# manhtuando97/two-stage-gnn

Hardware: AMD Instinct MI355X
Metric: graphs/sec fwd+bwd, DD batch=32 SAGE-3L h=128 (higher is better)
Workload: dtype f32

## Files before the change

include/tsgnn.h:

```cpp
#ifndef TSGNN_H
#define TSGNN_H
#include <stdint.h>

typedef struct ihipStream_t* tsgnn_stream_t;

#ifdef __cplusplus
extern "C" {
#endif

#define TSGNN_ABI_VERSION 2
int tsgnn_abi_version(void);
const char* tsgnn_strerror(int code);
const char* tsgnn_last_kernel(void);


int tsgnn_scan_workspace_ints(int64_t n, int64_t* ws_ints);
int tsgnn_exclusive_scan_i32(const int* in, int64_t n, int* out, int* ws, tsgnn_stream_t stream);

int tsgnn_row_maps(const int* graph_ptr, int B, int64_t n_rows, int* row_graph, int* row_slot,
                   tsgnn_stream_t stream);

int tsgnn_dense_adj_count(const float* adj, int B, int nmax, const int* graph_ptr, const int* row_graph,
                          int64_t n_rows, int* row_cnt, tsgnn_stream_t stream);
int tsgnn_dense_adj_fill(const float* adj, int B, int nmax, const int* graph_ptr, const int* row_graph,
// ... 41 lines not shown
int tsgnn_collate_pool_submit(tsgnn_collate_pool* pool, const int64_t* ds_graph_ptr, const int64_t* ds_rowptr, const int64_t* ds_col,
                              const int64_t* ds_node_label, const int64_t* ds_graph_label, const int64_t* ids, int B, int nmax,
                              int64_t row_cap, int64_t edge_cap, int ell_w, int64_t tail_cap, int32_t* staging, int64_t* out,
                              void* after_event, int64_t* ticket);
int tsgnn_collate_pool_submit_ack(tsgnn_collate_pool* pool, const int64_t* ds_graph_ptr, const int64_t* ds_rowptr, const int64_t* ds_col,
                                  const int64_t* ds_node_label, const int64_t* ds_graph_label, const int64_t* ids, int B, int nmax,
                                  int64_t row_cap, int64_t edge_cap, int ell_w, int64_t tail_cap, int32_t* staging, int64_t* out,
                                  const int64_t* host_ack, int64_t ack_target, int seq, int64_t* ticket);
int tsgnn_collate_pool_wait(tsgnn_collate_pool* pool, int64_t ticket);
int tsgnn_collate_pool_destroy(tsgnn_collate_pool* pool);

int tsgnn_csr_transpose(const int* rowptr, const int* col, const float* val, int64_t n_rows, int64_t n_cols,
                        int64_t nnz, int* rowptr_t, int* col_t, float* val_t, int* src_e, int* cnt_ws,
                        int* scan_ws, tsgnn_stream_t stream);


int tsgnn_csr_spmm_f32(const int* rowptr, const int* col, const float* val, const float* self_w,
                       const float* x, int64_t ldx, float* y, int64_t ldy, int64_t n_rows, int feat,
                       float self_scalar, int relu_in, int accumulate, tsgnn_stream_t stream);

int tsgnn_csr_to_ell(const int* rowptr, const int* col, int64_t n_rows, int W, int* ell, int* tail_cnt, tsgnn_stream_t stream);
int tsgnn_csr_tail_fill(const int* rowptr, const int* col, const int* tail_ptr, int64_t n_rows, int W, int* tail_col,
                        tsgnn_stream_t stream);
int tsgnn_ell_spmm_f32(const int* ell, int W, const float* x, int64_t ldx, float* y, int64_t ldy, int64_t n_rows, int feat,
                       float self_scalar, tsgnn_stream_t stream);

int tsgnn_gcn_norm_f32(const int* rowptr, const int* col, const float* val, int64_t n_rows, float self_fill,
                       float* dinv, float* val_out, float* self_w, tsgnn_stream_t stream);

int tsgnn_sddmm_rows_f32(const int* rowptr, const int* col, const float* dy, int64_t lddy, const float* x, int64_t ldx,
                         int64_t n_rows, int feat, float* dval, float* dself, tsgnn_stream_t stream);


int tsgnn_gemm_f32(const float* A, int64_t sam, int64_t sak, const float* B, int64_t sbk, int64_t sbn, float* C,
                   int64_t scm, int64_t scn, int M, int N, int K, int batch, int64_t stride_a, int64_t stride_b,
                   int64_t stride_c, const int* seg_ptr, int ragged, int max_seg, float alpha, int accumulate,
                   tsgnn_stream_t stream);
int tsgnn_gemm_splitk_plan(int M, int N, int K, int* ksplit, int64_t* ws_floats);
int tsgnn_gemm_splitk_f32(const float* A, int64_t sam, int64_t sak, const float* B, int64_t sbk, int64_t sbn,
                          float* C, int M, int N, int K, int ksplit, float* ws, int accumulate,
                          tsgnn_stream_t stream);
int tsgnn_linear_wgrad_plan(int64_t rows, int K_in, int N, int64_t ldz, int64_t lddu, int* nslab, int64_t* rows_per_slab,
                            int64_t* ws_floats);
int tsgnn_linear_wgrad_f32(const float* z, int64_t ldz, const float* du, int64_t lddu, int64_t rows, int K_in, int N, int nslab,
                           int64_t rows_per_slab, int64_t bias_only_rows, float* ws, float* dw, float* db, tsgnn_stream_t stream);
int tsgnn_wgrad_reduce_sets_blocks(const int64_t* desc);
int tsgnn_wgrad_reduce_sets_f32(const int64_t* desc, float* normparts, float* step_state, tsgnn_stream_t stream);
int tsgnn_wgrad_reduce_multi_f32(const float* ws0, int nslab0, int K0, int N0, float* dw0, float* db0, const float* ws1, int nslab1,
                                 int K1, int N1, float* dw1, float* db1, const float* ws2, int nslab2, int K2, int N2, float* dw2,
                                 float* db2, const float* ws3, int nslab3, int K3, int N3, float* dw3, float* db3,
                                 float* normparts, float* step_state, tsgnn_stream_t stream);
int tsgnn_wgrad_blocks_plan(int64_t rows, int K_in, int N, int64_t ldz, int64_t lddu, int* nslab, int64_t* rows_per_slab,
                            int64_t* ws_floats);
int tsgnn_wgrad_blocks_f32(const float* z, int64_t ldz, const float* du, int64_t lddu, int64_t rows, int K_in, int N, int nslab,
                           int64_t rows_per_slab, float* ws, float* dw, int64_t lddw, tsgnn_stream_t stream);
int tsgnn_wgrad_blocks_oi_f32(const float* z, int64_t ldz, const float* du, int64_t lddu, int64_t rows, int K_in, int N, int nslab,
                              int64_t rows_per_slab, float* ws, float* dw_oi, int64_t lddw, float* db, tsgnn_stream_t stream);
int tsgnn_ragged_tn_f32(const float* s_mat, int64_t lds_, const float* x, int64_t ldx, int K, int N, const int* slab_row_ptr,
                        int nslab, const int* seg_slab_ptr, int nseg, float* ws, float* out, tsgnn_stream_t stream);
int tsgnn_ragged_tn_direct_supported(int K, int64_t max_rows);
int tsgnn_ragged_tn_direct_f32(const float* s_mat, int64_t lds_, int K, const int* graph_ptr, int B, const float* x0, int64_t ldx0,
                               int N0, float* out0, const float* x1, int64_t ldx1, int N1, float* out1, tsgnn_stream_t stream);
int tsgnn_ragged_tn_direct_ro_f32(const float* s_mat, int64_t lds_, int K, const int* graph_ptr, int B, const float* x0, int64_t ldx0,
                                  int N0, float* out0, const float* x1, int64_t ldx1, int N1, float* out1, float* ro_out,
                                  int64_t ro_ldo, int* ro_arg, int nmax, int64_t n_real, int ghost_zero, tsgnn_stream_t stream);
int tsgnn_wgrad_narrow_plan(int64_t rows, int K_in, int N, int64_t* ws_floats);
int tsgnn_wgrad_narrow_f32(const float* z, int64_t ldz, const float* du, int64_t lddu, int64_t rows, int K_in, int N, float* ws,
                           float* dwb, tsgnn_stream_t stream);
int tsgnn_colsum_f32(const float* x, int64_t ld, int64_t rows, int F, float* out, float* ws, int accumulate,
                     tsgnn_stream_t stream);

int tsgnn_linear_l2norm_f32(const float* z, int64_t ldz, const float* w, int64_t ldw, const float* bias, float* v,
                            int64_t ldv, float* rinv, int64_t rows, int K, int N, int normalize,
                            tsgnn_stream_t stream);
int tsgnn_rowgemm_supported(const float* a, int64_t lda, const float* b, int64_t ldb, const float* c, int64_t ldc, int K, int N,
                            int trans_b);
int tsgnn_rowgemm_f32(const float* a, int64_t lda, const float* b, int64_t ldb, int trans_b, const float* bias, float* c,
                      int64_t ldc, float* rinv, int64_t rows, int K, int N, int normalize, int64_t fill_rows,
                      tsgnn_stream_t stream);
int tsgnn_panel_blocks(int64_t rows, int panel_units);
int tsgnn_gather_rowgemm_f32(const int* ell, int ell_w, const int* tail_ptr, const int* tail_col, const float* x, int64_t ldx, const float* b, int64_t ldb, int trans_b,
                             const float* bias, float* c, int64_t ldc, float* rinv, float* zout, int64_t ldz, int64_t rows, int K,
                             int N, int normalize, int64_t fill_rows, tsgnn_stream_t stream);
int tsgnn_gather_rowgemm_st_f32(const int* ell, int ell_w, const int* tail_ptr, const int* tail_col, const float* x, int64_t ldx, const float* b, int64_t ldb, const float* bias,
                                float* c, int64_t ldc, float* rinv, float* zout, int64_t ldz, int64_t rows, int K, int N,
                                int64_t fill_rows, const int* row_slot, unsigned long long* sums, float* ghost, int panel_units,
                                const int64_t* pack_desc, tsgnn_stream_t stream);
int tsgnn_sage_layer_fwd_bn_f32(const int* ell, int ell_w, const int* tail_ptr, const int* tail_col, const float* x, int64_t ldx, const float* w, int64_t ldw, const float* bias,
                                float* v, int64_t ldv, float* rinv, float* zout, int64_t ldz, int64_t rows, int K, int64_t fill_rows,
                                const int* graph_ptr, const int* slot_count, int B, int nslots, int n_ghost, unsigned long long* packed,
                                unsigned long long* packed_out, const int* row_graph, const unsigned long long* sums_in,
                                const float* ghost_in, float* mean_out, float* rstd_out, const int* row_slot,
                                unsigned long long* sums_out, float* ghost_out, const int* ro_map, int ro_map_ch, int panel_units,
                                const float* w_img, tsgnn_stream_t stream);
int tsgnn_sage_layer_fwd_bn_plan(int64_t rows, int64_t fill_rows, int B, int nslots, int panel_units, int* ro_ch, int* n_gemm,
                                 int* n_full);
int tsgnn_sage_layer_fwd_f32(const int* ell, int ell_w, const int* tail_ptr, const int* tail_col, const float* x, int64_t ldx, const float* w, int64_t ldw, const float* bias,
                             float* v, int64_t ldv, float* rinv, float* zout, int64_t ldz, int64_t rows, int K, int64_t fill_rows,
                             const int* graph_ptr, int B, int nslots, int n_ghost, unsigned long long* packed, tsgnn_stream_t stream);
int tsgnn_sage_layer_fwd_ro_f32(const int* ell, int ell_w, const int* tail_ptr, const int* tail_col, const float* x, int64_t ldx, const float* w, int64_t ldw, const float* bias,
                                float* v, int64_t ldv, float* rinv, float* zout, int64_t ldz, int64_t rows, int K, int64_t fill_rows,
                                const int* graph_ptr, int B, int nslots, int n_ghost, unsigned long long* packed,
                                unsigned long long* packed_out, const int* row_graph, tsgnn_stream_t stream);
int tsgnn_sage_layer_bwd_f32(const int* ell, int ell_w, const int* tail_ptr, const int* tail_col, const float* du, int64_t lddu, const float* w, int64_t ldw, float* dxs,
                             int64_t lddxs, const float* z, int64_t ldz, int64_t rows, int nslab, int64_t rows_per_slab,
                             int64_t bias_only_rows, float* ws, int panel_units, const float* w_img, tsgnn_stream_t stream);
int tsgnn_l2norm_bwd_f32(const float* v, int64_t ldv, const float* dv, int64_t lddv, const float* rinv, float* du,
                         int64_t lddu, int64_t rows, int F, tsgnn_stream_t stream);


int tsgnn_bn_slots_fwd_f32(const int* graph_ptr, const int* slot_count, const int* row_slot, int B, int nmax,
                           int64_t n_real, int n_ghost, const float* v, int64_t ldv, int F, int relu, int bn,
                           float* mean, float* rstd, float* y, int64_t ldy, tsgnn_stream_t stream);
int tsgnn_bn_slots_bwd_f32(const int* graph_ptr, const int* slot_count, const int* row_slot, int B, int nmax,
                           int64_t n_real, int n_ghost, const float* v, int64_t ldv, const float* dy, int64_t lddy, int F,
                           int relu, int bn, const float* mean, const float* rstd, float* m1, float* m2, float* dv,
                           int64_t lddv, tsgnn_stream_t stream);

int tsgnn_row_ln_fwd_f32(const float* v, int64_t ldv, int64_t rows, int F, int relu, float* mean, float* rstd, float* y, int64_t ldy,
                         tsgnn_stream_t stream);
int tsgnn_row_ln_bwd_f32(const float* v, int64_t ldv, const float* dy, int64_t lddy, int64_t rows, int F, int relu, const float* mean,
                         const float* rstd, float* dv, int64_t lddv, tsgnn_stream_t stream);

int tsgnn_row_post_bwd_f32(const int* row_graph, int B, int64_t n_real, int64_t rows, const float* v, int64_t ldv, const float* dxs,
                           int64_t lddxs, const float* dout, int64_t ldo, const int* arg, int F, int relu, int ln, const float* mean,
                           const float* rstd, const float* rinv, float* du, int64_t lddu, tsgnn_stream_t stream);

int tsgnn_row_post_nodes_bwd_f32(int64_t n_real, int64_t rows, const float* v, int64_t ldv, const float* dxs, int64_t lddxs,
                                 const float* dnode, int64_t lddn, int ghost_zero, int F, int relu, int ln, const float* mean,
                                 const float* rstd, const float* rinv, float* du, int64_t lddu, tsgnn_stream_t stream);

int tsgnn_readout_max_ws_words(int B, int nmax, int F);
int tsgnn_readout_max_fwd_f32(const int* graph_ptr, const int* slot_count, int B, int nmax, int64_t n_real, int n_ghost,
                              const float* x, int64_t ldx, int F, int relu, unsigned long long* packed_ws, float* out,
                              int64_t ldo, int* arg, tsgnn_stream_t stream);
int tsgnn_readout_max_bwd_f32(const float* dout, int64_t ldo, const int* arg, int B, int F, const float* x, int64_t ldx_in,
                              int relu, int64_t n_real, float* dx, int64_t ldx, tsgnn_stream_t stream);
int tsgnn_readout_max_bwd_rows_f32(const float* dout, int64_t ldo, const int* arg, const int* row_graph, int F, int64_t rows,
                                   int64_t rows_total, const float* add, int64_t ldadd, float* dx, int64_t ldx, tsgnn_stream_t stream);

int tsgnn_pack_rows_f32(const float* src, int nmax, int F, const int* row_graph, const int* row_slot, int64_t n_real,
                        float* dst, int64_t ld, tsgnn_stream_t stream);
int tsgnn_unpack_rows_f32(const int* graph_ptr, int B, int nmax, int64_t n_real, int n_ghost, const float* src, int64_t ld,
                          int F, float fill, float* dst, tsgnn_stream_t stream);
int tsgnn_unpack_rows_bwd_ghost_f32(const int* graph_ptr, int B, int nmax, int64_t n_real, const float* ddst, int F,
                                    float* dsrc, int64_t ld, tsgnn_stream_t stream);


int tsgnn_softmax_ce_f32(const float* logits, int64_t ld, const int64_t* label, int B, int C, float* loss, float* dlogits,
                         tsgnn_stream_t stream);
int tsgnn_adam_from_partials_f32(float* param, const float* grad, float* m, float* v, int64_t n, float lr, float beta1, float beta2,
                                 float eps, float weight_decay, float max_norm, float* state, const float* parts, int nparts,
                                 const float* poison, tsgnn_stream_t stream);
int tsgnn_clip_adam_step_f32(float* param, const float* grad, float* m, float* v, int64_t n, float lr, float beta1,
                             float beta2, float eps, float weight_decay, float max_norm, float grad_scale, float* state,
                             float* ws, const float* poison, tsgnn_stream_t stream);


int tsgnn_dense_stack_supported(int B, int K, int nstack, int L, int fin0, int hidden, int last0, int last1);
int tsgnn_dense_stack_fwd_f32(const int64_t* desc, tsgnn_stream_t stream);
int tsgnn_dense_stack_bwd_f32(const int64_t* desc, tsgnn_stream_t stream);
int tsgnn_dense_stack_max_resident(void);
int tsgnn_dense_stack_barrier_selftest(unsigned* sync, float* err, int expect, tsgnn_stream_t stream);


int tsgnn_node_scores_f32(const float* x, int64_t ldx, int64_t rows, int H, int Fh, const float* a, int64_t lda, float* s,
                          tsgnn_stream_t stream);
int tsgnn_node_scores2_f32(const float* x, int64_t ldx, int64_t rows, int H, int Fh, const float* a1, int64_t lda1, float* s1,
                           const float* a2, int64_t lda2, float* s2, tsgnn_stream_t stream);
int tsgnn_edge_softmax_fwd_f32(const int* rowptr, const int* col, int64_t rows, int H, const float* s_grp, const float* s_oth,
                               int mod, float slope, float* alpha, tsgnn_stream_t stream);
int tsgnn_edge_softmax_bwd_f32(const int* rowptr, const int* col, int64_t rows, int H, const float* s_grp, const float* s_oth,
                               int mod, float slope, const float* alpha, const float* dalpha, float* dt, float* ds_grp,
                               tsgnn_stream_t stream);
int tsgnn_edge_permute_f32(const float* src, const int* perm, int64_t n, int H, int scatter, float* dst, tsgnn_stream_t stream);
int tsgnn_csr_row_sum_f32(const int* rowptr, const float* val, int64_t rows, int H, float* out, tsgnn_stream_t stream);
int tsgnn_csr_row_sum_perm_f32(const int* rowptr, const float* val, const int* eperm, int64_t rows, int H, float* out,
                               tsgnn_stream_t stream);
int tsgnn_csr_spmm_heads_f32(const int* rowptr, const int* col, const float* alpha, int H, int Fh, const float* x, int64_t ldx,
                             int mod, float* y, int64_t ldy, int64_t rows, tsgnn_stream_t stream);
int tsgnn_csr_spmm_heads_epi_f32(const int* rowptr, const int* col, const float* alpha, int H, int Fh, const float* x, int64_t ldx,
                                 int mod, float* y, int64_t ldy, int64_t rows, const float* w1, const float* a1, int64_t lda1,
                                 const float* w2, const float* a2, int64_t lda2, const float* u, int64_t ldu, const float* uw,
                                 int rows_per_seg, const int* row_seg, float uscale, const int* eperm, tsgnn_stream_t stream);
int tsgnn_csr_sddmm_heads_f32(const int* rowptr, const int* col, int H, int Fh, const float* dy, int64_t lddy, const float* x,
                              int64_t ldx, int mod, float* dalpha, int64_t rows, tsgnn_stream_t stream);
int tsgnn_segment_wsum_f32(const float* x, int64_t ldx, const float* w, int H, int Fh, const int* seg_ptr, int nseg, int64_t rows,
                           int64_t max_seg, float scale, int mean, float* ws, float* out, int64_t ldo, tsgnn_stream_t stream);
int tsgnn_segment_wsum2_f32(const float* x, int64_t ldx, const float* w1, const float* w2, int H, int Fh, const int* seg_ptr, int nseg,
                            int64_t rows, int64_t max_seg, float scale, float* ws, float* out1, float* out2, int64_t ldo,
                            tsgnn_stream_t stream);
int tsgnn_gather_wsum_f32(const float* x, int64_t ldx, const int* idx, const float* w, const int* seg_ptr, int nseg, int C, float scale,
                          float* out, int64_t ldo, tsgnn_stream_t stream);
int tsgnn_broadcast_add_f32(float* y, int64_t ldy, int64_t rows, int H, int Fh, const float* w, const float* a, int64_t lda,
                            const float* u, int64_t ldu, int rows_per_seg, float scale, tsgnn_stream_t stream);
int tsgnn_pack_heads_max(void);
int tsgnn_pack_heads_f32(const float* w0, const float* w1, const float* w2, const float* w3, const float* w4, const float* w5,
                         const float* w6, const float* w7, const float* a0, const float* a1, const float* a2, const float* a3,
                         const float* a4, const float* a5, const float* a6, const float* a7, int H, int Fin, int Fo, float* W, float* A,
                         tsgnn_stream_t stream);
int tsgnn_unpack_heads_f32(const float* dW, const float* dA0, const float* dA1, int H, int Fin, int Fo, float* gw, float* ga,
                           tsgnn_stream_t stream);

int tsgnn_gat_fused_supported(int H, int Fh);
int tsgnn_gat_attn_fwd_f32(const float* hp, int64_t ldh, const int* rowptr, const int* col, const int* rp_t, const int* col_t,
                           int64_t rows, int H, int Fh, float slope, const int* row_graph, int nmax, const int* iso_idx,
                           const float* iso_w, const int* iso_ptr, float uscale, int mean_heads, int apply_elu, float drop_p,
                           uint64_t seed, const unsigned long long* drop_ctr, float* stat, float* y, int64_t ldy, tsgnn_stream_t stream);
int tsgnn_gat_bwd_parts(int B);
int tsgnn_gat_attn_bwd_f32(const float* hp, int64_t ldh, const float* y, int64_t ldy, const float* dy, int64_t lddy, const int* rp_t,
                           const int* col_t, int64_t rows, int H, int Fh, float slope, int mean_heads, int apply_elu,
                           const int* graph_ptr, int B, const int* iso_idx, const float* iso_w, const int* iso_ptr,
                           const float* iso_row, int iso_row_ld, float uscale, float drop_p, uint64_t seed,
                           const unsigned long long* drop_ctr, const float* stat, float* dhp, int Ns, float* t1, float* t2, float* S,
                           float* dupart, tsgnn_stream_t stream);
int tsgnn_gat_attn_bwd_ro_f32(const float* hp, int64_t ldh, const float* y, int64_t ldy, const float* dy, int64_t lddy, const int* rp_t,
                              const int* col_t, int64_t rows, int H, int Fh, float slope, int mean_heads, int apply_elu,
                              const int* graph_ptr, int B, const int* iso_idx, const float* iso_w, const int* iso_ptr,
                              const float* iso_row, int iso_row_ld, float uscale, float drop_p, uint64_t seed,
                              const unsigned long long* drop_ctr, const float* stat, float* dhp, int Ns, float* t1, float* t2, float* S,
                              float* dupart, const float* ro_dout, int64_t ro_ldo, const int* ro_arg, const int* row_graph,
                              tsgnn_stream_t stream);
int tsgnn_gat_dropout_mult_f32(float drop_p, uint64_t seed, const unsigned long long* drop_ctr, int64_t i0, int64_t ni, int64_t j0,
                               int64_t nj, int H, float* out, tsgnn_stream_t stream);
int tsgnn_gat_score_rowsum_f32(const int* rowptr, const int* col, const int* eperm, const float* t1, const float* t2, const float* S,
                               int64_t rows, int H, float* dhp, int64_t ldh, int C, const float* dupart, int B, const int* iso_idx,
                               const float* iso_w, const int* iso_ptr, float uscale, tsgnn_stream_t stream);
int tsgnn_gat_pack_desc_words(void);
int tsgnn_gat_pack_f32(const int64_t* desc, tsgnn_stream_t stream);
int tsgnn_gat_unpack_f32(const int64_t* desc, tsgnn_stream_t stream);
int tsgnn_elu_heads_fwd_f32(const float* x, int64_t rows, int H, int Fh, int mean_heads, int apply_elu, float* y, tsgnn_stream_t stream);
int tsgnn_elu_heads_bwd_f32(const float* x, const float* dy, int64_t rows, int H, int Fh, int mean_heads, int apply_elu, float* dx,
                            tsgnn_stream_t stream);


int tsgnn_mlp3_supported(int B, int D0, int D1, int D2, int C);
int tsgnn_mlp3_fwd_f32(const float* x, int64_t ldx, const float* w1, const float* b1, const float* keep, float keep_scale, const float* w2,
                       const float* b2, const float* w3, const float* b3, int B, int D0, int D1, int D2, int C, float* a1, float* a2,
                       float* logp, tsgnn_stream_t stream);
int tsgnn_mlp3_fwd_drop_f32(const float* x, int64_t ldx, const float* w1, const float* b1, float p, uint64_t seed,
                            unsigned long long* state, unsigned long long* used, const float* w2, const float* b2, const float* w3,
                            const float* b3, int B, int D0, int D1, int D2, int C, float* a1, float* a2, float* logp,
                            tsgnn_stream_t stream);
int tsgnn_mlp3_dropout_mask_f32(float p, uint64_t seed, uint64_t counter, int B, int D1, float* out, tsgnn_stream_t stream);
int tsgnn_mlp3_bwd_f32(const float* x, int64_t ldx, const float* w1, const float* w2, const float* w3, const float* a1,
                       const float* a2, const float* logp, const float* dlogp, float keep_scale, int B, int D0, int D1, int D2, int C,
                       float* dw1, float* db1, float* dw2, float* db2, float* dw3, float* db3, float* dx, int64_t lddx,
                       tsgnn_stream_t stream);
int tsgnn_mlp3_bwd2_f32(const float* x, int64_t ldx, const float* w1, const float* w2, const float* w3, const float* a1,
                        const float* a2, const float* logp, const float* dlogp, float keep_scale, int B, int D0, int D1, int D2, int C,
                        float* dw1, float* db1, float* dw2, float* db2, float* dw3, float* db3, float* dx, int64_t lddx, float* ws,
                        tsgnn_stream_t stream);
int tsgnn_mlp3_bwd2_nll_f32(const float* x, int64_t ldx, const float* w1, const float* w2, const float* w3, const float* a1,
                            const float* a2, const float* logp, const int64_t* label, float* loss, float keep_scale, int B, int D0,
                            int D1, int D2, int C, float* dw1, float* db1, float* dw2, float* db2, float* dw3, float* db3, float* dx,
                            int64_t lddx, float* ws, tsgnn_stream_t stream);

int tsgnn_mlp3_bwd2_norm_blocks(int D1, int D2);
int tsgnn_mlp3_bwd2_np_f32(const float* x, int64_t ldx, const float* w1, const float* w2, const float* w3, const float* a1,
                           const float* a2, const float* logp, const float* dlogp, const int64_t* label, float* loss, float keep_scale, int B,
                           int D0, int D1, int D2, int C, float* dw1, float* db1, float* dw2, float* db2, float* dw3, float* db3, float* dx,
                           int64_t lddx, float* ws, float* normparts, tsgnn_stream_t stream);

int tsgnn_mlp3_triplet_supported(int D0, int D1, int D2, int C);
int tsgnn_mlp3_triplet_fwd_f32(const float* x, int64_t ldx, const float* w1, const float* b1, float p, uint64_t seed,
                               unsigned long long* state, unsigned long long* used, const float* w2, const float* b2, const float* w3,
                               const float* b3, int D0, int D1, int D2, int C, float eps, float* a1, float* a2, float* embed, float* dist,
                               tsgnn_stream_t stream);
int tsgnn_mlp3_triplet_bwd_f32(const float* x, int64_t ldx, const float* w1, const float* w2, const float* w3, const float* a1,
                               const float* a2, const float* embed, const float* dist, float eps, float keep_scale, const float* g_dp,
                               const float* g_dn, const float* g_ea, const float* g_ep, const float* g_en, int D0, int D1, int D2, int C,
                               float* dw1, float* db1, float* dw2, float* db2, float* dw3, float* db3, float* dx, int64_t lddx,
                               tsgnn_stream_t stream);


int tsgnn_linkpred_tile_rows(void);
int tsgnn_linkpred_chunks(void);
int tsgnn_linkpred_loss_f32(const float* S, int64_t lds, int K, int64_t rows, const int* slab_row_ptr, const int* slab_graph,
                            int nslab, const int* graph_ptr, const int* rowptr, const int* col, const float* val,
                            const int* rowptr_t, const int* col_t, const float* val_t, float clamp, float inv_entries, float* dS,
                            int64_t ldd, float* ws, float* part, float* loss, tsgnn_stream_t stream);
int tsgnn_linkpred_loss_xy_f32(const float* X, int64_t ldx, const float* Y, int64_t ldy, int K, int64_t rows, const int* slab_row_ptr,
                               const int* slab_graph, int nslab, const int* graph_ptr, const int* rowptr, const int* col,
                               const float* val, float clamp, float inv_entries, int count_loss, float* dX, int64_t ldd, float* ws,
                               float* part, float* loss, tsgnn_stream_t stream);


int tsgnn_topk_max_segment(void);
int tsgnn_topk_segments_f32(const float* score, const int* graph_ptr, const int* k_ptr, int B, int max_seg, int* perm,
                            int* new_id, tsgnn_stream_t stream);
int tsgnn_gather_gate_fwd_f32(const float* x, int64_t ldx, const float* score, const int* perm, int64_t K, int F, int use_tanh,
                              float* out, int64_t ldo, tsgnn_stream_t stream);
int tsgnn_gather_gate_bwd_f32(const float* x, int64_t ldx, const float* score, const int* perm, int64_t K, int F, int use_tanh,
                              const float* dout, int64_t ldo, float* dx, int64_t lddx, float* dscore, tsgnn_stream_t stream);
int tsgnn_filter_edges_mark(const int* perm, int64_t K, int64_t N, const int64_t* src, const int64_t* dst, int64_t E,
                            int* new_id, int* flag, tsgnn_stream_t stream);
int tsgnn_filter_edges_compact(const int64_t* src, const int64_t* dst, int64_t E, const int* new_id, const int* flag,
                               const int* pos, int64_t* out_src, int64_t* out_dst, int64_t* kept_eid, tsgnn_stream_t stream);
int tsgnn_gcn_coef_f32(const int* rowptr, const int* col, int64_t n_rows, float* dinv, float* self_w, tsgnn_stream_t stream);
int tsgnn_gcn_propagate_f32(const int* rowptr, const int* col, const float* dinv, const float* self_w, const float* x,
                            int64_t ldx, int relu_in, const float* bias, const float* w_dot, const float* dot_bias, float* y,
                            int64_t ldy, float* t, int64_t n_rows, int feat, tsgnn_stream_t stream);
int tsgnn_gcn_propagate_re_f32(const int* rowptr, const int* rowend, const int* col, const float* dinv, const float* self_w,
                               const float* x, int64_t ldx, int relu_in, const float* bias, const float* w_dot, const float* dot_bias,
                               float* y, int64_t ldy, float* t, int64_t n_rows, int feat, tsgnn_stream_t stream);
int tsgnn_gcn_propagate_affine_f32(const int* rowptr, const int* rowend, const int* col, const float* dinv, const float* self_w,
// ... 238 lines not shown
```

two-stage-gnn_amd/csrc/dense_stack.hip:

```cpp
#include "common.h"
#include <utility>
#include "../../include/tsgnn.h"

#ifdef TSGNN_TRACE_BWD
#define TRF(x) do { } while (0)
#define TRB(x) TR(x)
#else
#define TRF(x) TR(x)
#define TRB(x) do { } while (0)
#endif

namespace {

constexpr int DS_TR = 16;
#ifndef TSGNN_DS_THREADS
#define TSGNN_DS_THREADS 512
#endif
constexpr int DS_NT = TSGNN_DS_THREADS;
constexpr int DS_NW = DS_NT / 64;
static_assert(DS_NT == 256 || DS_NT == 512, "main threads are the first 256");
constexpr int DS_MAXL = 4;
constexpr int DS_BIG = 15360;
constexpr float DS_NORM_EPS = 1e-12f;
constexpr float DS_BN_EPS = 1e-5f;

struct DsLayer {
  const float* w; int64_t ldw; const float* bias; int fin, n, off;
  float* agg;
  float* v;
  float* rinv;
  float* mean; float* rstd;
  float* dw; float* db;
  int64_t slab_off;
};
struct DsStack { float* out; int64_t ldo; const float* dout; int64_t lddo; int L; DsLayer layer[DS_MAXL]; };
struct DsArgs {
  const float* x; int64_t ldx; int fin0; const float* adj; int B, K, nstack;
  DsStack st[2];
  float* stats;
  float* dagg;
  float* dxn;
  float* slabs;
  int64_t slab_floats; int finmax;
  float* dx; int64_t lddx; float* dadj;
  float* dadj_part;
  const float* dadj_add;
  unsigned* sync; float* err;
};

__device__ __forceinline__ void drain_stores() { asm volatile("s_waitcnt vmcnt(0)" ::: "memory"); }
template <bool LIGHT = false>
__device__ __forceinline__ void grid_barrier(unsigned* words, int& k, unsigned nblocks, float* err) {
  drain_stores();
  __syncthreads();
  if (threadIdx.x == 0) {
    if (LIGHT) __hip_atomic_fetch_add(words + k, 1u, __ATOMIC_RELAXED, __HIP_MEMORY_SCOPE_AGENT);
    else __hip_atomic_fetch_add(words + k, 1u, __ATOMIC_RELEASE, __HIP_MEMORY_SCOPE_AGENT);
    bool ok = false;
    for (int spin = 0; spin < (1 << 21); ++spin) {
      if (__hip_atomic_load(words + k, __ATOMIC_RELAXED, __HIP_MEMORY_SCOPE_AGENT) >= nblocks) { ok = true; break; }
      __builtin_amdgcn_s_sleep(2);
    }
    if (!LIGHT) __builtin_amdgcn_fence(__ATOMIC_ACQUIRE, "agent");
    if (!ok) __hip_atomic_store(err, 1.0f, __ATOMIC_RELAXED, __HIP_MEMORY_SCOPE_AGENT);
    if (k > 0 && blockIdx.x == 0) __hip_atomic_store(words + k - 1, 0u, __ATOMIC_RELAXED, __HIP_MEMORY_SCOPE_AGENT);
  }
  ++k;
  __syncthreads();
}
template <bool LIGHT = false>
__device__ __forceinline__ void grid_arrive(unsigned* words, int k) {
  drain_stores();
  __syncthreads();
  if (threadIdx.x == 0) {
    if (LIGHT) __hip_atomic_fetch_add(words + k, 1u, __ATOMIC_RELAXED, __HIP_MEMORY_SCOPE_AGENT);
    else __hip_atomic_fetch_add(words + k, 1u, __ATOMIC_RELEASE, __HIP_MEMORY_SCOPE_AGENT);
  }
}
template <bool LIGHT = false>
__device__ __forceinline__ void grid_wait(unsigned* words, int& k, unsigned nblocks, float* err) {
  if (threadIdx.x == 0) {
    bool ok = false;
    for (int spin = 0; spin < (1 << 21); ++spin) {
      if (__hip_atomic_load(words + k, __ATOMIC_RELAXED, __HIP_MEMORY_SCOPE_AGENT) >= nblocks) { ok = true; break; }
      __builtin_amdgcn_s_sleep(2);
    }
    if (!LIGHT) __builtin_amdgcn_fence(__ATOMIC_ACQUIRE, "agent");
    if (!ok) __hip_atomic_store(err, 1.0f, __ATOMIC_RELAXED, __HIP_MEMORY_SCOPE_AGENT);
    if (k > 0 && blockIdx.x == 0) __hip_atomic_store(words + k - 1, 0u, __ATOMIC_RELAXED, __HIP_MEMORY_SCOPE_AGENT);
  }
  ++k;
  __syncthreads();
}
__device__ __forceinline__ void group_barrier(unsigned* word, unsigned target, float* err) {
  drain_stores();
  __syncthreads();
  if (threadIdx.x == 0) {
    __hip_atomic_fetch_add(word, 1u, __ATOMIC_RELEASE, __HIP_MEMORY_SCOPE_AGENT);
    bool ok = false;
    for (int spin = 0; spin < (1 << 21); ++spin) {
      if (__hip_atomic_load(word, __ATOMIC_RELAXED, __HIP_MEMORY_SCOPE_AGENT) >= target) { ok = true; break; }
      __builtin_amdgcn_s_sleep(1);
    }
    __builtin_amdgcn_fence(__ATOMIC_ACQUIRE, "agent");
    if (!ok) __hip_atomic_store(err, 1.0f, __ATOMIC_RELAXED, __HIP_MEMORY_SCOPE_AGENT);
  }
  __syncthreads();
}
__device__ __forceinline__ void ds_put2(float* p, float x, float y) {
  const unsigned long long bits = ((unsigned long long)__float_as_uint(y) << 32) | (unsigned long long)__float_as_uint(x);
  __hip_atomic_store(reinterpret_cast<unsigned long long*>(p), bits, __ATOMIC_RELAXED, __HIP_MEMORY_SCOPE_AGENT);
}
__device__ __forceinline__ float2 ds_get2(const float* p) {
  const unsigned long long bits = __hip_atomic_load(reinterpret_cast<const unsigned long long*>(p), __ATOMIC_RELAXED, __HIP_MEMORY_SCOPE_AGENT);
  return make_float2(__uint_as_float((unsigned)(bits & 0xffffffffull)), __uint_as_float((unsigned)(bits >> 32)));
}
__device__ __forceinline__ void grid_finish(unsigned* words, int k, unsigned nblocks) {
  if (threadIdx.x == 0 && k > 0) {
    const unsigned prev = __hip_atomic_fetch_add(words + 31, 1u, __ATOMIC_ACQ_REL, __HIP_MEMORY_SCOPE_AGENT);
    if (prev == nblocks - 1) {
      __hip_atomic_store(words + k - 1, 0u, __ATOMIC_RELAXED, __HIP_MEMORY_SCOPE_AGENT);
      __hip_atomic_store(words + 31, 0u, __ATOMIC_RELAXED, __HIP_MEMORY_SCOPE_AGENT);
    }
  }
}

struct FastDiv {
  float inv; int d;
  __device__ __forceinline__ explicit FastDiv(int d_) : inv(1.0f / (float)d_), d(d_) {}
  __device__ __forceinline__ int operator()(int x) const {
    int q = (int)(((float)x + 0.5f) * inv);
    const int r = x - q * d;
    q += (r >= d) - (r < 0);
    return q;
  }
};

template <bool TRANSPOSE, typename F>
__device__ __forceinline__ void fill_lds(float* lds, int lds_ld, const float* __restrict__ g, int64_t ldg, int rows, int cols, F f) {
  const int tid = threadIdx.x;
  const int c4n = cols >> 2, total = rows * c4n;
  const FastDiv by_c4n(c4n);
  for (int base = tid; base < total; base += 8 * DS_NT) {
    float4 v[8];
    int rr[8], cc[8];
#pragma unroll
    for (int u = 0; u < 8; ++u) {
      const int idx = base + u * DS_NT;
      rr[u] = by_c4n(idx); cc[u] = 4 * (idx - rr[u] * c4n);
      v[u] = idx < total ? *reinterpret_cast<const float4*>(g + (int64_t)rr[u] * ldg + cc[u]) : make_float4(0.f, 0.f, 0.f, 0.f);
    }
#pragma unroll
    for (int u = 0; u < 8; ++u) {
      if (base + u * DS_NT < total) {
        const float o0 = f(v[u].x, rr[u], cc[u]), o1 = f(v[u].y, rr[u], cc[u] + 1), o2 = f(v[u].z, rr[u], cc[u] + 2), o3 = f(v[u].w, rr[u], cc[u] + 3);
        if (TRANSPOSE) {
          lds[(cc[u] + 0) * lds_ld + rr[u]] = o0; lds[(cc[u] + 1) * lds_ld + rr[u]] = o1;
          lds[(cc[u] + 2) * lds_ld + rr[u]] = o2; lds[(cc[u] + 3) * lds_ld + rr[u]] = o3;
        } else {
          *reinterpret_cast<float4*>(lds + rr[u] * lds_ld + cc[u]) = make_float4(o0, o1, o2, o3);
        }
      }
    }
  }
}
struct Ident { __device__ __forceinline__ float operator()(float v, int, int) const { return v; } };

template <int NV>
struct Pf { float4 v[NV]; };
template <typename F, int... I>
__device__ __forceinline__ void pf_each(F&& f, std::integer_sequence<int, I...>) { (f(std::integral_constant<int, I>{}), ...); }
template <int NV>
__device__ __forceinline__ void pf_load(Pf<NV>& p, const float* __restrict__ g, int64_t ldg, int rows, int cols) {
  const int c4n = cols >> 2, total = rows * c4n;
  const FastDiv by_c4n(c4n);
  pf_each([&](auto u) {
    const int idx = min(u.value * DS_NT + (int)threadIdx.x, total - 1);
    const int rr = by_c4n(idx), cc = 4 * (idx - rr * c4n);
    p.v[u.value] = *reinterpret_cast<const float4*>(g + (int64_t)rr * ldg + cc);
  }, std::make_integer_sequence<int, NV>{});
}
template <int NV, bool TRANSPOSE>
__device__ __forceinline__ void pf_store(float* lds, int lds_ld, const Pf<NV>& p, int rows, int cols) {
  const int c4n = cols >> 2, total = rows * c4n;
  const FastDiv by_c4n(c4n);
  pf_each([&](auto u) {
    const int idx = u.value * DS_NT + (int)threadIdx.x;
    if (idx < total) {
      const int rr = by_c4n(idx), cc = 4 * (idx - rr * c4n);
      const float4 v = p.v[u.value];
      if (TRANSPOSE) {
        lds[(cc + 0) * lds_ld + rr] = v.x; lds[(cc + 1) * lds_ld + rr] = v.y;
        lds[(cc + 2) * lds_ld + rr] = v.z; lds[(cc + 3) * lds_ld + rr] = v.w;
      } else {
        *reinterpret_cast<float4*>(lds + rr * lds_ld + cc) = v;
      }
    }
  }, std::make_integer_sequence<int, NV>{});
}
constexpr int DS_PFW = (15360 / 4 + DS_NT - 1) / DS_NT;
__device__ __forceinline__ void zero_lds(float* lds, int n) {
  for (int i = threadIdx.x; i < n; i += DS_NT) lds[i] = 0.f;
}
__device__ __forceinline__ int pad64(int n) { return (n + 63) & ~63; }

typedef float f32x4 __attribute__((ext_vector_type(4)));

__device__ __forceinline__ void tile_mfma(float* c, int ldc, const float* a, int ars, int acs, const float* bm, int ldb, int depth, int ng) {
  const int lane = threadIdx.x & 63, w = threadIdx.x >> 6;
  const int i = lane & 15, kq = lane >> 4;
  const int steps = depth >> 2;
  for (int g = w; g < ng; g += DS_NW) {
    f32x4 acc = {0.f, 0.f, 0.f, 0.f};
    if ((steps & 15) == 0) {
      const float* ap = a + i * ars + kq * acs;
      const float* bp = bm + kq * ldb + 16 * g + i;
      auto load16 = [&](int s0, float (&af)[16], float (&bf)[16]) {
#pragma unroll
        for (int u = 0; u < 16; ++u) { af[u] = ap[4 * (s0 + u) * acs]; bf[u] = bp[4 * (s0 + u) * ldb]; }
      };
      float a0[16], b0[16], a1[16], b1[16];
      load16(0, a0, b0);
      for (int s0 = 0;; s0 += 32) {
        const bool more1 = s0 + 16 < steps;
        load16(more1 ? s0 + 16 : 0, a1, b1);
#pragma unroll
        for (int u = 0; u < 16; ++u) acc = __builtin_amdgcn_mfma_f32_16x16x4f32(a0[u], b0[u], acc, 0, 0, 0);
        if (!more1) break;
        const bool more2 = s0 + 32 < steps;
        load16(more2 ? s0 + 32 : 0, a0, b0);
#pragma unroll
        for (int u = 0; u < 16; ++u) acc = __builtin_amdgcn_mfma_f32_16x16x4f32(a1[u], b1[u], acc, 0, 0, 0);
        if (!more2) break;
      }
    } else
    for (int s0 = 0; s0 < steps; s0 += 16) {
      float af[16], bf[16];
#pragma unroll
      for (int u = 0; u < 16; ++u) {
        const int k = 4 * (s0 + u) + kq;
        const bool ok = s0 + u < steps;
        af[u] = ok ? a[i * ars + k * acs] : 0.f;
        bf[u] = ok ? bm[k * ldb + 16 * g + i] : 0.f;
      }
#pragma unroll
      for (int u = 0; u < 16; ++u) acc = __builtin_amdgcn_mfma_f32_16x16x4f32(af[u], bf[u], acc, 0, 0, 0);
    }
#pragma unroll
    for (int v = 0; v < 4; ++v) c[(4 * kq + v) * ldc + 16 * g + i] = acc[v];
  }
}
__device__ __forceinline__ void zero_acc(float (&acc)[3][4]) {
#pragma unroll
  for (int j = 0; j < 3; ++j)
#pragma unroll
    for (int q = 0; q < 4; ++q) acc[j][q] = 0.f;
}
__device__ __forceinline__ void read_tile(float (&acc)[3][4], const float* tile, int ld, int r, int cg, int J) {
#pragma unroll
  for (int j = 0; j < 3; ++j) {
    const float4 v = j < J ? *reinterpret_cast<const float4*>(tile + r * ld + 4 * cg + 64 * j) : make_float4(0.f, 0.f, 0.f, 0.f);
    acc[j][0] = v.x; acc[j][1] = v.y; acc[j][2] = v.z; acc[j][3] = v.w;
  }
}
__device__ __forceinline__ void slot_totals(const float* st, int B, int K, int n, float& t1, float& t2) {
  t1 = 0.f; t2 = 0.f;
  int bb = 0;
  for (; bb + 8 <= B; bb += 8) {
    float2 v[8];
#pragma unroll
    for (int u = 0; u < 8; ++u) v[u] = ds_get2(st + ((int64_t)(bb + u) * K + n) * 2);
#pragma unroll
    for (int u = 0; u < 8; ++u) { t1 += v[u].x; t2 += v[u].y; }
  }
  for (; bb < B; ++bb) { const float2 v = ds_get2(st + ((int64_t)bb * K + n) * 2); t1 += v.x; t2 += v.y; }
}

// ... 589 lines not shown
```

two-stage-gnn_amd/csrc/gemm.hip:

```cpp
#include "common.h"
#include <algorithm>
#include <cstdlib>
#include <type_traits>
#include "../../include/tsgnn.h"

#include "tn_rows_body.h"
#include "wgrad_blocks_body.h"
#include "du_reduce_body.h"

namespace {

typedef float f32x16 __attribute__((ext_vector_type(16)));

constexpr int BM = 64, BN = 64, BK = 32;
constexpr int LDA_S = BK + 1;
constexpr int LDB_S = BN + 1;

struct GemmArgs {
  const float* A; const float* B; float* C;
  int64_t sam, sak, sbk, sbn, scm, scn;
  int64_t stride_a, stride_b, stride_c;
  int M, N, K;
  const int* seg_ptr;
  int ragged;
  int ksplit;
  int64_t slab_stride;
  float alpha;
  int accumulate;
};

__global__ __launch_bounds__(256) void gemm_f32_kernel(GemmArgs g) {
  __shared__ float As[BM * LDA_S];
  __shared__ float Bs[BK * LDB_S];
  const int z = blockIdx.z;
  const int tile_n = blockIdx.x, tile_m = blockIdx.y / g.ksplit, split = blockIdx.y % g.ksplit;
  const float* A = g.A + (int64_t)z * g.stride_a;
  const float* B = g.B + (int64_t)z * g.stride_b;
  float* C = g.C + (int64_t)z * g.stride_c + (int64_t)split * g.slab_stride;
  int M = g.M, K = g.K;
  if (g.seg_ptr) {
    const int s0 = g.seg_ptr[z], s1 = g.seg_ptr[z + 1];
    if (g.ragged == 1) { A += (int64_t)s0 * g.sak; B += (int64_t)s0 * g.sbk; K = s1 - s0; }
    else { A += (int64_t)s0 * g.sam; C += (int64_t)s0 * g.scm; M = s1 - s0; }
  }
  const int m0 = tile_m * BM, n0 = tile_n * BN;
  if (m0 >= M) return;
  const int kchunks = (K + BK - 1) / BK;
  const int per = (kchunks + g.ksplit - 1) / g.ksplit;
  const int kbeg = split * per * BK;
  const int kend = min(K, (split + 1) * per * BK);

  const int tid = threadIdx.x, lane = tid & 63, wid = tid >> 6;
  const int wr = wid >> 1, wc = wid & 1;
  f32x16 acc;
#pragma unroll
  for (int i = 0; i < 16; ++i) acc[i] = 0.f;

  const bool a_k_fast = (g.sak == 1);
  const bool b_n_fast = (g.sbn == 1);
  constexpr int AV = (BM * BK) / 256, BV = (BK * BN) / 256;
  float ra[AV], rb[BV];
  auto fetch = [&](int k0) {
#pragma unroll
    for (int it = 0; it < AV; ++it) {
      const int idx = it * 256 + tid;
      int m, k;
      if (a_k_fast) { m = idx / BK; k = idx % BK; } else { k = idx / BM; m = idx % BM; }
      const int gm = m0 + m, gk = k0 + k;
      ra[it] = (gm < M && gk < kend) ? A[(int64_t)gm * g.sam + (int64_t)gk * g.sak] : 0.f;
    }
#pragma unroll
    for (int it = 0; it < BV; ++it) {
      const int idx = it * 256 + tid;
      int k, n;
      if (b_n_fast) { k = idx / BN; n = idx % BN; } else { n = idx / BK; k = idx % BK; }
      const int gk = k0 + k, gn = n0 + n;
      rb[it] = (gk < kend && gn < g.N) ? B[(int64_t)gk * g.sbk + (int64_t)gn * g.sbn] : 0.f;
    }
  };
  auto commit = [&]() {
#pragma unroll
    for (int it = 0; it < AV; ++it) {
      const int idx = it * 256 + tid;
      int m, k;
      if (a_k_fast) { m = idx / BK; k = idx % BK; } else { k = idx / BM; m = idx % BM; }
      As[m * LDA_S + k] = ra[it];
    }
#pragma unroll
    for (int it = 0; it < BV; ++it) {
      const int idx = it * 256 + tid;
      int k, n;
      if (b_n_fast) { k = idx / BN; n = idx % BN; } else { n = idx / BK; k = idx % BK; }
      Bs[k * LDB_S + n] = rb[it];
    }
  };
  if (kbeg < kend) fetch(kbeg);
  for (int k0 = kbeg; k0 < kend; k0 += BK) {
    commit();
    __syncthreads();
    const int i = lane & 31, h = lane >> 5;
    const float* ap = As + (wr * 32 + i) * LDA_S + h;
    const float* bp = Bs + h * LDB_S + wc * 32 + i;
    float af[BK / 2], bf[BK / 2];
#pragma unroll
    for (int kk = 0; kk < BK; kk += 2) { af[kk / 2] = ap[kk]; bf[kk / 2] = bp[kk * LDB_S]; }
    __builtin_amdgcn_sched_barrier(0);
    if (k0 + BK < kend) fetch(k0 + BK);
    __builtin_amdgcn_sched_barrier(0);
#pragma unroll
    for (int j = 0; j < BK / 2; ++j) acc = __builtin_amdgcn_mfma_f32_32x32x2f32(af[j], bf[j], acc, 0, 0, 0);
    __syncthreads();
  }
  const int cn = n0 + wc * 32 + (lane & 31);
  if (cn < g.N) {
#pragma unroll
    for (int r = 0; r < 16; ++r) {
      const int cm = m0 + wr * 32 + (r & 3) + 8 * (r >> 2) + 4 * (lane >> 5);
      if (cm < M) {
        float* cp = C + (int64_t)cm * g.scm + (int64_t)cn * g.scn;
        const float v = g.alpha * acc[r];
        *cp = (g.accumulate && g.ksplit == 1) ? (*cp + v) : v;
      }
    }
  }
}

__global__ void splitk_reduce_kernel(const float* __restrict__ slabs, int nsplit, int64_t slab_stride, int64_t n,
                                     float* __restrict__ out, int accumulate) {
  int64_t i = (int64_t)blockIdx.x * blockDim.x + threadIdx.x;
  if (i >= n) return;
  float s = accumulate ? out[i] : 0.f;
  int k = 0;
  for (; k + 8 <= nsplit; k += 8) {
    float t[8];
#pragma unroll
    for (int u = 0; u < 8; ++u) t[u] = slabs[(int64_t)(k + u) * slab_stride + i];
    s += ((t[0] + t[1]) + (t[2] + t[3])) + ((t[4] + t[5]) + (t[6] + t[7]));
  }
  for (; k < nsplit; ++k) s += slabs[(int64_t)k * slab_stride + i];
  out[i] = s;
}

__global__ __launch_bounds__(256) void colsum_partial(const float* __restrict__ x, int64_t ld, int64_t rows, int F,
                                                      int64_t rows_per_chunk, float* __restrict__ part) {
  __shared__ float lds[4][64];
  const int f = blockIdx.x * 64 + (threadIdx.x & 63);
  const int rl = threadIdx.x >> 6;
  const int64_t r0 = (int64_t)blockIdx.y * rows_per_chunk, r1 = min(rows, r0 + rows_per_chunk);
  float s = 0.f;
  if (f < F) {
    int64_t r = r0 + rl;
    for (; r + 28 < r1; r += 32) {
      float t[8];
#pragma unroll
      for (int u = 0; u < 8; ++u) t[u] = x[(r + 4 * u) * ld + f];
      s += ((t[0] + t[1]) + (t[2] + t[3])) + ((t[4] + t[5]) + (t[6] + t[7]));
    }
    for (; r < r1; r += 4) s += x[r * ld + f];
  }
  lds[rl][threadIdx.x & 63] = s;
  __syncthreads();
  if (rl == 0 && f < F) part[(int64_t)blockIdx.y * F + f] = lds[0][threadIdx.x] + lds[1][threadIdx.x] + lds[2][threadIdx.x] + lds[3][threadIdx.x];
}


constexpr int WN_KMAX = 4;
__global__ __launch_bounds__(256) void wgrad_narrow_partial(const float* __restrict__ z, int64_t ldz, const float* __restrict__ du,
                                                            int64_t lddu, int64_t rows, int K_in, int F, int64_t rows_per_chunk,
                                                            float* __restrict__ part) {
  __shared__ float lds[WN_KMAX + 1][4][64];
  const int fl = threadIdx.x & 63, f = blockIdx.x * 64 + fl;
  const int rl = threadIdx.x >> 6;
  const int64_t r0 = (int64_t)blockIdx.y * rows_per_chunk, r1 = min(rows, r0 + rows_per_chunk);
  float acc[WN_KMAX + 1];
#pragma unroll
  for (int k = 0; k <= WN_KMAX; ++k) acc[k] = 0.f;
  if (f < F) {
    for (int64_t rb = r0 + rl; rb < r1; rb += 32) {
      float t[8], zz[8][WN_KMAX];
#pragma unroll
      for (int u = 0; u < 8; ++u) {
        const int64_t r = rb + 4 * u;
        const bool ok = r < r1;
        t[u] = ok ? du[r * lddu + f] : 0.f;
#pragma unroll
        for (int k = 0; k < WN_KMAX; ++k) zz[u][k] = (ok && k < K_in) ? z[r * ldz + k] : 0.f;
      }
#pragma unroll
      for (int u = 0; u < 8; ++u) {
#pragma unroll
        for (int k = 0; k < WN_KMAX; ++k) acc[k] = fmaf(zz[u][k], t[u], acc[k]);
        acc[WN_KMAX] += t[u];
      }
    }
  }
#pragma unroll
  for (int k = 0; k <= WN_KMAX; ++k) lds[k][rl][fl] = acc[k];
  __syncthreads();
  if (rl == 0 && f < F) {
    float* o = part + (int64_t)blockIdx.y * (K_in + 1) * F;
    for (int k = 0; k < K_in; ++k) o[(int64_t)k * F + f] = (lds[k][0][fl] + lds[k][1][fl]) + (lds[k][2][fl] + lds[k][3][fl]);
    o[(int64_t)K_in * F + f] = (lds[WN_KMAX][0][fl] + lds[WN_KMAX][1][fl]) + (lds[WN_KMAX][2][fl] + lds[WN_KMAX][3][fl]);
  }
}

template <int MT, int NTt, int NY>
__global__ __launch_bounds__(256) void gemm_tn_rows_kernel(TnArgs g) {
  extern __shared__ __attribute__((aligned(16))) float tn_smem[];
  tn_rows_body<MT, NTt, NY>(g, tn_smem, blockIdx.x, blockIdx.y, gridDim.x);
}

__device__ __forceinline__ float slab_sum(const float* __restrict__ slabs, int nslab, int64_t per_slab, int64_t e, bool ok,
                                          float (*lds)[64]) {
  const int e_l = threadIdx.x & 63, grp = threadIdx.x >> 6;
  float a0 = 0.f, a1 = 0.f, a2 = 0.f, a3 = 0.f;
  if (ok) {
    const int per = (nslab + 3) / 4;
    const int s0 = grp * per, s1 = min(nslab, s0 + per);
    int s = s0;
    for (; s + 4 <= s1; s += 4) {
      a0 += slabs[(int64_t)s * per_slab + e];
      a1 += slabs[(int64_t)(s + 1) * per_slab + e];
      a2 += slabs[(int64_t)(s + 2) * per_slab + e];
      a3 += slabs[(int64_t)(s + 3) * per_slab + e];
    }
    for (; s < s1; ++s) a0 += slabs[(int64_t)s * per_slab + e];
  }
  lds[grp][e_l] = (a0 + a1) + (a2 + a3);
  __syncthreads();
  return (lds[0][e_l] + lds[1][e_l]) + (lds[2][e_l] + lds[3][e_l]);
}

__global__ __launch_bounds__(256) void tn_rows_reduce(const float* __restrict__ slabs, int64_t per_slab, int64_t n_w, float* __restrict__ out,
                                                      const int* __restrict__ seg_slab_ptr) {
  __shared__ float lds[4][64];
  const int64_t e = (int64_t)blockIdx.x * 64 + (threadIdx.x & 63);
  const int sb = seg_slab_ptr[blockIdx.y], se = seg_slab_ptr[blockIdx.y + 1];
  const float v = slab_sum(slabs + (int64_t)sb * per_slab, se - sb, per_slab, e, e < per_slab, lds);
  if (threadIdx.x < 64 && e < n_w) out[(int64_t)blockIdx.y * n_w + e] = v;
}

__global__ __launch_bounds__(256) void tn_rows_reduce_du(const float* __restrict__ slabs, int nslab, int64_t per_slab, int64_t n_w,
                                                         float* __restrict__ dw, float* __restrict__ db, float* __restrict__ part, int nb,
                                                         int F_du, float* __restrict__ dws, float* __restrict__ dbs) {
  __shared__ float4 s_part[256];
  if (blockIdx.x == gridDim.x - 1) {
    du_reduce_body(part, nb, F_du, dws, dbs, nb, 1, 0, s_part);
    return;
  }
  const int64_t e = (int64_t)blockIdx.x * 64 + (threadIdx.x & 63);
  const float v = slab_sum(slabs, nslab, per_slab, e, e < per_slab, reinterpret_cast<float (*)[64]>(s_part));
  if (threadIdx.x < 64 && e < per_slab) {
    if (e < n_w) dw[e] = v;
    else if (db) db[e - n_w] = v;
  }
}

struct ReduceSet {
  const float* ws; int nslab, K, N;
  float* dw; int64_t lddw; int kn;
  float* db; int n_db; float* tail;
};
constexpr int RM_SETS = 12;
struct ReduceMulti { int first_block[RM_SETS]; ReduceSet s[RM_SETS]; int n; float* normparts; float* step_state; };

__global__ __launch_bounds__(256) void tn_rows_reduce_multi(ReduceMulti m) {
  __shared__ float lds[4][64];
  int si = 0;
#pragma unroll
  for (int t = 1; t < RM_SETS; ++t) if (t < m.n && (int)blockIdx.x >= m.first_block[t]) si = t;
  const ReduceSet& r = m.s[si];
  const int e_l = threadIdx.x & 63;
  const int64_t per_slab = (int64_t)(r.K + 1) * r.N;
  const int64_t e = (int64_t)((int)blockIdx.x - m.first_block[si]) * 64 + e_l;
  const float v = slab_sum(r.ws, r.nslab, per_slab, e, e < per_slab, lds);
  if (threadIdx.x >= 64) return;
  float sq = 0.f;
  if (e < per_slab) {
    const int k = (int)e / r.N, n = (int)e % r.N;
    if (k < r.K) { r.dw[r.kn ? (int64_t)k * r.lddw + n : (int64_t)n * r.lddw + k] = v; sq = v * v; }
    else if (r.db && n < r.n_db) { r.db[n] = v; sq = v * v; }
    else if (r.tail && n == r.n_db) { r.tail[0] = v; sq = v * v; }
    else if (r.K == 0 && r.dw && n >= r.lddw && n < r.lddw + r.n_db) { r.dw[n - r.lddw] = v; sq = v * v; }
  }
  if (m.normparts) {
    sq = wave_sum(sq);
    if (e_l == 0) m.normparts[blockIdx.x] = sq;
  }
  if (m.step_state && blockIdx.x == 0 && e_l == 0) m.step_state[0] += 1.f;
}

template <int NY>
__global__ __launch_bounds__(256) void wgrad_blocks_kernel(WgradBlocks w) {
  extern __shared__ __attribute__((aligned(16))) float tn_smem[];
  wgrad_blocks_role<NY>(w, tn_smem, blockIdx.x, blockIdx.y, gridDim.x);
}
}

constexpr int RS_WORDS = 11;
struct ReducePlan { ReduceSet s[RM_SETS * WB_MAXSETS]; int64_t first_block[RM_SETS * WB_MAXSETS + 1]; int n; };

static int reduce_plan(const int64_t* desc, ReducePlan& p) {
  if (!desc || desc[0] < 0 || desc[0] > RM_SETS) return TSGNN_EINVAL;
  p.n = 0;
  p.first_block[0] = 0;
  auto add = [&p](const ReduceSet& r) {
    p.first_block[p.n + 1] = p.first_block[p.n] + ceil_div64((int64_t)(r.K + 1) * r.N, 64);
    p.s[p.n++] = r;
  };
  for (int t = 0; t < (int)desc[0]; ++t) {
    const int64_t* d = desc + 1 + RS_WORDS * t;
    const float* ws = reinterpret_cast<const float*>(d[0]);
    const int64_t nslab = d[1], K = d[2], N = d[3], lddw = d[5], n_db = d[7], kn = d[9], blocked = d[10];
    float* dw = reinterpret_cast<float*>(d[4]);
    float* db = reinterpret_cast<float*>(d[6]);
    float* tail = reinterpret_cast<float*>(d[8]);
    if (!ws || nslab <= 0 || nslab > INT32_MAX || K < 0 || N <= 0 || (K + 1) * N > INT32_MAX || n_db < 0 || n_db > N) return TSGNN_EINVAL;
    if ((kn != 0 && kn != 1) || (blocked != 0 && blocked != 1)) return TSGNN_EINVAL;
    if (K > 0 && (!dw || lddw < (kn ? N : K))) return TSGNN_EINVAL;
    if (tail && n_db >= N) return TSGNN_EINVAL;
    if (K == 0 && dw && (lddw <= n_db || lddw + n_db > N)) return TSGNN_EINVAL;
    if (!blocked) {
      add(ReduceSet{ws, (int)nslab, (int)K, (int)N, dw, lddw, (int)kn, db, (int)n_db, tail});
      continue;
    }
    const int KB = (int)(K + 127) / 128, NB = (int)(N + 127) / 128;
    if (K == 0 || K > 512 || N > 512 || KB * NB > WB_MAXSETS || tail || (db && n_db != N)) return TSGNN_EINVAL;
    for (int kb = 0; kb < KB; ++kb)
      for (int nb = 0; nb < NB; ++nb) {
        const int kc = (int)std::min<int64_t>(128, K - 128 * kb), nc = (int)std::min<int64_t>(128, N - 128 * nb);
        float* dwb = dw + (kn ? 128 * kb * lddw + 128 * nb : 128 * nb * lddw + 128 * kb);
        add(ReduceSet{ws + (kb * NB + nb) * nslab * WB_SET_FLOATS, (int)nslab, kc, nc, dwb, lddw, (int)kn, (db && kb == 0) ? db + 128 * nb : nullptr,
                      nc, nullptr});
      }
  }
  return TSGNN_OK;
}

static int reduce_launch(const ReducePlan& p, float* normparts, float* step_state, tsgnn_stream_t stream) {
  for (int i = 0; i < p.n; i += RM_SETS) {
    ReduceMulti m{};
    m.n = std::min(RM_SETS, p.n - i);
    const int64_t b0 = p.first_block[i], b1 = p.first_block[i + m.n];
    for (int t = 0; t < m.n; ++t) {
      m.s[t] = p.s[i + t];
      m.first_block[t] = (int)(p.first_block[i + t] - b0);
    }
    m.normparts = normparts ? normparts + b0 : nullptr;
    m.step_state = i == 0 ? step_state : nullptr;
    tn_rows_reduce_multi<<<(unsigned)(b1 - b0), 256, 0, stream>>>(m);
  }
  TSGNN_CHECK_LAUNCH();
  return TSGNN_OK;
}

static int reduce_one(const float* ws, int nslab, int K, int N, float* dw, int64_t lddw, int kn, float* db, int blocked, tsgnn_stream_t stream) {
  const int64_t desc[1 + RS_WORDS] = {1, (int64_t)(uintptr_t)ws, nslab, K, N, (int64_t)(uintptr_t)dw, lddw, (int64_t)(uintptr_t)db, N, 0, kn,
                                      blocked};
  ReducePlan p;
  const int rc = reduce_plan(desc, p);
  return rc != TSGNN_OK ? rc : reduce_launch(p, nullptr, nullptr, stream);
}

extern "C" {

int tsgnn_gemm_f32(const float* A, int64_t sam, int64_t sak, const float* B, int64_t sbk, int64_t sbn, float* C,
                   int64_t scm, int64_t scn, int M, int N, int K, int batch, int64_t stride_a, int64_t stride_b,
                   int64_t stride_c, const int* seg_ptr, int ragged, int max_seg, float alpha, int accumulate,
                   tsgnn_stream_t stream) {
  if (!A || !B || !C || M < 0 || N < 0 || K < 0 || batch <= 0) return TSGNN_EINVAL;
  if (seg_ptr && ragged != 1 && ragged != 2) return TSGNN_EINVAL;
  if (!seg_ptr && ragged != 0) return TSGNN_EINVAL;
  const int Mgrid = (seg_ptr && ragged == 2) ? max_seg : M;
  if (Mgrid <= 0 || N == 0) return TSGNN_OK;
  GemmArgs g{A, B, C, sam, sak, sbk, sbn, scm, scn, stride_a, stride_b, stride_c, M, N, K, seg_ptr, ragged, 1, 0,
             alpha, accumulate};
  dim3 grid((unsigned)((N + BN - 1) / BN), (unsigned)((Mgrid + BM - 1) / BM), (unsigned)batch);
  gemm_f32_kernel<<<grid, 256, 0, stream>>>(g);
  TSGNN_CHECK_LAUNCH();
  return TSGNN_OK;
}

int tsgnn_gemm_splitk_plan(int M, int N, int K, int* ksplit, int64_t* ws_floats) {
  if (!ksplit || !ws_floats || M < 0 || N < 0 || K < 0) return TSGNN_EINVAL;
  const int tiles = ((M + BM - 1) / BM) * ((N + BN - 1) / BN);
  const int kchunks = (K + BK - 1) / BK;
  int s = tiles > 0 ? (1024 + tiles - 1) / tiles : 1;
  if (s > kchunks / 4) s = kchunks / 4;
  if (s < 1) s = 1;
  if (s > 256) s = 256;
  *ksplit = s;
  *ws_floats = (s > 1) ? (int64_t)s * M * N : 0;
  return TSGNN_OK;
}

int tsgnn_gemm_splitk_f32(const float* A, int64_t sam, int64_t sak, const float* B, int64_t sbk, int64_t sbn,
                          float* C, int M, int N, int K, int ksplit, float* ws, int accumulate,
                          tsgnn_stream_t stream) {
  if (!A || !B || !C || M <= 0 || N <= 0 || K < 0 || ksplit < 1 || (ksplit > 1 && !ws)) return TSGNN_EINVAL;
  GemmArgs g{A, B, ksplit > 1 ? ws : C, sam, sak, sbk, sbn, (int64_t)N, 1, 0, 0, 0, M, N, K, nullptr, 0, ksplit,
             (int64_t)M * N, 1.f, accumulate};
  dim3 grid((unsigned)((N + BN - 1) / BN), (unsigned)(((M + BM - 1) / BM) * ksplit), 1);
  gemm_f32_kernel<<<grid, 256, 0, stream>>>(g);
  if (ksplit > 1) {
    const int64_t n = (int64_t)M * N;
    splitk_reduce_kernel<<<(unsigned)ceil_div64(n, 256), 256, 0, stream>>>(ws, ksplit, n, n, C, accumulate);
  }
  TSGNN_CHECK_LAUNCH();
  return TSGNN_OK;
}


int tsgnn_linear_wgrad_plan(int64_t rows, int K_in, int N, int64_t ldz, int64_t lddu, int* nslab, int64_t* rows_per_slab,
                            int64_t* ws_floats) {
  if (!nslab || !rows_per_slab || !ws_floats || rows < 0) return TSGNN_EINVAL;
  *nslab = 0; *rows_per_slab = 0; *ws_floats = 0;
  if (K_in <= 0 || N <= 0 || K_in > 128 || N > 128 || (ldz % 4) || (lddu % 4) || (N % 4)) return TSGNN_OK;
  const int ncu = device_cu_count();
  const int tiles = ((K_in + 31) / 32) * ((N + 31) / 32);
  const int per_slab_blocks = tiles >= 8 ? 2 : 1;
  int64_t rps = ceil_div64(rows > 0 ? rows : 1, ncu / per_slab_blocks);
  rps = ((rps + 7) / 8) * 8;
  if (rps < 16) rps = 16;
  *rows_per_slab = rps;
  *nslab = (int)(rows > 0 ? ceil_div64(rows, rps) : 1);
  *ws_floats = (int64_t)(*nslab) * (K_in + 1) * N;
  return TSGNN_OK;
}

int tsgnn_wgrad_reduce_multi_f32(const float* ws0, int nslab0, int K0, int N0, float* dw0, float* db0, const float* ws1, int nslab1,
                                 int K1, int N1, float* dw1, float* db1, const float* ws2, int nslab2, int K2, int N2, float* dw2,
                                 float* db2, const float* ws3, int nslab3, int K3, int N3, float* dw3, float* db3,
                                 float* normparts, float* step_state, tsgnn_stream_t stream) {
  const float* ws[4] = {ws0, ws1, ws2, ws3};
  const int ns[4] = {nslab0, nslab1, nslab2, nslab3}, Ks[4] = {K0, K1, K2, K3}, Ns[4] = {N0, N1, N2, N3};
  float* dws[4] = {dw0, dw1, dw2, dw3};
  float* dbs[4] = {db0, db1, db2, db3};
  int64_t desc[1 + 4 * RS_WORDS] = {0};
  for (int t = 0; t < 4; ++t) {
    if (!ws[t]) continue;
    if (Ks[t] <= 0) return TSGNN_EINVAL;
    const int64_t r[RS_WORDS] = {(int64_t)(uintptr_t)ws[t], ns[t], Ks[t], Ns[t], (int64_t)(uintptr_t)dws[t], Ns[t], (int64_t)(uintptr_t)dbs[t],
                                 Ns[t], 0, 1, 0};
    std::copy(r, r + RS_WORDS, desc + 1 + RS_WORDS * desc[0]++);
  }
  return tsgnn_wgrad_reduce_sets_f32(desc, normparts, step_state, stream);
}

static int linear_wgrad_launch(const float* z, int64_t ldz, const float* du, int64_t lddu, int64_t rows, int K_in, int N, int nslab,
                               int64_t rows_per_slab, int64_t bias_only_rows, float* ws, float* dw, float* db, float* du_part, int du_nb,
                               int du_F, float* du_dws, float* du_dbs, tsgnn_stream_t stream) {
  if (!z || !du || !ws || rows < 0 || nslab <= 0 || rows_per_slab <= 0 || K_in <= 0 || N <= 0 || bias_only_rows < 0) return TSGNN_EINVAL;
  if (K_in > 128 || N > 128 || (ldz % 4) || (lddu % 4) || (N % 4) || (reinterpret_cast<uintptr_t>(z) & 15) ||
      (reinterpret_cast<uintptr_t>(du) & 15))
    return TSGNN_EUNSUPPORTED;
  TnArgs g{z, ldz, du, lddu, rows, rows_per_slab, K_in, N, ws, nullptr, bias_only_rows};
  const int mt = (K_in + 31) / 32, nt = (N + 31) / 32;
  const int tiles = mt * nt;
  const unsigned ny = (tiles >= 8 && nslab < 512) ? 2u : 1u;
  const dim3 grid_tn((unsigned)nslab, ny);
  TSGNN_KNAME("gemm_tn_rows_kernel<%d,%d,%u>", mt > 4 ? 4 : mt, nt > 4 ? 4 : nt, ny);
#define TSGNN_TN(M_, N_) do { if (ny == 2) gemm_tn_rows_kernel<M_, N_, 2><<<grid_tn, 256, 2 * TN_CH * 32 * (M_ + N_) * sizeof(float), stream>>>(g); \
    else gemm_tn_rows_kernel<M_, N_, 1><<<grid_tn, 256, 2 * TN_CH * 32 * (M_ + N_) * sizeof(float), stream>>>(g); } while (0)
  switch (mt * 10 + nt) {
    case 11: TSGNN_TN(1, 1); break; case 12: TSGNN_TN(1, 2); break; case 13: TSGNN_TN(1, 3); break; case 14: TSGNN_TN(1, 4); break;
    case 21: TSGNN_TN(2, 1); break; case 22: TSGNN_TN(2, 2); break; case 23: TSGNN_TN(2, 3); break; case 24: TSGNN_TN(2, 4); break;
    case 31: TSGNN_TN(3, 1); break; case 32: TSGNN_TN(3, 2); break; case 33: TSGNN_TN(3, 3); break; case 34: TSGNN_TN(3, 4); break;
    case 41: TSGNN_TN(4, 1); break; case 42: TSGNN_TN(4, 2); break; case 43: TSGNN_TN(4, 3); break; default: TSGNN_TN(4, 4); break;
  }
#undef TSGNN_TN
  if (dw && !du_part) return reduce_one(ws, nslab, K_in, N, dw, N, 1, db, 0, stream);
  const int64_t per_slab = (int64_t)(K_in + 1) * N;
  if (dw)
    tn_rows_reduce_du<<<(unsigned)ceil_div64(per_slab, 64) + 1, 256, 0, stream>>>(ws, nslab, per_slab, (int64_t)K_in * N, dw, db, du_part,
                                                                                   du_nb, du_F, du_dws, du_dbs);
  TSGNN_CHECK_LAUNCH();
  return TSGNN_OK;
}

int tsgnn_linear_wgrad_f32(const float* z, int64_t ldz, const float* du, int64_t lddu, int64_t rows, int K_in, int N, int nslab,
                           int64_t rows_per_slab, int64_t bias_only_rows, float* ws, float* dw, float* db, tsgnn_stream_t stream) {
  return linear_wgrad_launch(z, ldz, du, lddu, rows, K_in, N, nslab, rows_per_slab, bias_only_rows, ws, dw, db, nullptr, 0, 0, nullptr,
                             nullptr, stream);
}

int tsgnn_linear_wgrad_du_f32(const float* z, int64_t ldz, const float* du, int64_t lddu, int64_t rows, int K_in, int N, int nslab,
                              int64_t rows_per_slab, float* ws, float* dw, float* db, float* part, int nb, int F_du, float* dws,
                              float* dbs, tsgnn_stream_t stream) {
  if (!dw || !part || !dws || !dbs || nb <= 0 || nb > 256 || F_du <= 0 || (F_du % 4) || (reinterpret_cast<uintptr_t>(part) & 15) ||
      (reinterpret_cast<uintptr_t>(dws) & 15))
    return TSGNN_EINVAL;
  return linear_wgrad_launch(z, ldz, du, lddu, rows, K_in, N, nslab, rows_per_slab, 0, ws, dw, db, part, nb, F_du, dws, dbs, stream);
}


int tsgnn_ragged_tn_f32(const float* s_mat, int64_t lds_, const float* x, int64_t ldx, int K, int N, const int* slab_row_ptr,
                        int nslab, const int* seg_slab_ptr, int nseg, float* ws, float* out, tsgnn_stream_t stream) {
  if (!s_mat || !x || !slab_row_ptr || !seg_slab_ptr || !ws || !out || K <= 0 || N <= 0 || nslab <= 0 || nseg <= 0) return TSGNN_EINVAL;
  const int mt = (K + 31) / 32, nt = (N + 31) / 32;
  if (mt * nt > 16 || mt > 4 || nt > 8 || (lds_ % 4) || (ldx % 4) || (N % 4) || (reinterpret_cast<uintptr_t>(s_mat) & 15) ||
      (reinterpret_cast<uintptr_t>(x) & 15))
    return TSGNN_EUNSUPPORTED;
  TnArgs g{s_mat, lds_, x, ldx, 0, 0, K, N, ws, slab_row_ptr, 0};
  const unsigned ny = (mt * nt >= 8) ? 2u : 1u;
  const dim3 grid((unsigned)nslab, ny);
#define TSGNN_RT(M_, N_) do { if (ny == 2) gemm_tn_rows_kernel<M_, N_, 2><<<grid, 256, 2 * TN_CH * 32 * (M_ + N_) * sizeof(float), stream>>>(g); \
    else gemm_tn_rows_kernel<M_, N_, 1><<<grid, 256, 2 * TN_CH * 32 * (M_ + N_) * sizeof(float), stream>>>(g); } while (0)
  switch (mt * 10 + nt) {
    case 11: TSGNN_RT(1, 1); break; case 12: TSGNN_RT(1, 2); break; case 13: TSGNN_RT(1, 3); break; case 14: TSGNN_RT(1, 4); break;
    case 15: TSGNN_RT(1, 5); break; case 16: TSGNN_RT(1, 6); break; case 17: TSGNN_RT(1, 7); break; case 18: TSGNN_RT(1, 8); break;
    case 21: TSGNN_RT(2, 1); break; case 22: TSGNN_RT(2, 2); break; case 23: TSGNN_RT(2, 3); break; case 24: TSGNN_RT(2, 4); break;
    case 25: TSGNN_RT(2, 5); break; case 26: TSGNN_RT(2, 6); break; case 27: TSGNN_RT(2, 7); break; case 28: TSGNN_RT(2, 8); break;
    case 31: TSGNN_RT(3, 1); break; case 32: TSGNN_RT(3, 2); break; case 33: TSGNN_RT(3, 3); break; case 34: TSGNN_RT(3, 4); break;
    case 35: TSGNN_RT(3, 5); break;
    case 41: TSGNN_RT(4, 1); break; case 42: TSGNN_RT(4, 2); break; case 43: TSGNN_RT(4, 3); break; default: TSGNN_RT(4, 4); break;
  }
#undef TSGNN_RT
  const int64_t per_slab = (int64_t)(K + 1) * N;
  dim3 rgrid((unsigned)ceil_div64((int64_t)K * N, 64), (unsigned)nseg);
  tn_rows_reduce<<<rgrid, 256, 0, stream>>>(ws, per_slab, (int64_t)K * N, out, seg_slab_ptr);
  TSGNN_CHECK_LAUNCH();
  return TSGNN_OK;
}

int tsgnn_wgrad_narrow_plan(int64_t rows, int K_in, int N, int64_t* ws_floats) {
  if (!ws_floats || rows < 0 || K_in <= 0 || N <= 0) return TSGNN_EINVAL;
  const int64_t rpc = rows > 65536 ? 512 : 128;
  *ws_floats = (rows > 0 ? ceil_div64(rows, rpc) : 1) * (int64_t)(K_in + 1) * N;
  return TSGNN_OK;
}

int tsgnn_wgrad_narrow_f32(const float* z, int64_t ldz, const float* du, int64_t lddu, int64_t rows, int K_in, int N, float* ws,
                           float* dwb, tsgnn_stream_t stream) {
  if (!dwb || rows < 0 || K_in <= 0 || N <= 0) return TSGNN_EINVAL;
  if (K_in > WN_KMAX) return TSGNN_EUNSUPPORTED;
  if (rows == 0) {
    (void)hipMemsetAsync(dwb, 0, sizeof(float) * (size_t)(K_in + 1) * N, stream);
    return TSGNN_OK;
  }
  if (!z || !du || !ws || ldz < K_in || lddu < N) return TSGNN_EINVAL;
  const int64_t rpc = rows > 65536 ? 512 : 128;
  const int nchunk = (int)(rows > 0 ? ceil_div64(rows, rpc) : 1);
  const int64_t n = (int64_t)(K_in + 1) * N;
  wgrad_narrow_partial<<<dim3((unsigned)((N + 63) / 64), (unsigned)nchunk), 256, 0, stream>>>(z, ldz, du, lddu, rows, K_in, N, rpc, ws);
  splitk_reduce_kernel<<<(unsigned)ceil_div64(n, 256), 256, 0, stream>>>(ws, nchunk, n, n, dwb, 0);
  TSGNN_CHECK_LAUNCH();
  return TSGNN_OK;
}

int tsgnn_colsum_f32(const float* x, int64_t ld, int64_t rows, int F, float* out, float* ws, int accumulate,
                     tsgnn_stream_t stream) {
  if (!x || !out || !ws || rows < 0 || F <= 0 || ld < F) return TSGNN_EINVAL;
  const int64_t rpc = rows > 65536 ? 512 : 128;
  const int nchunk = (int)(rows > 0 ? ceil_div64(rows, rpc) : 1);
  dim3 grid((unsigned)((F + 63) / 64), (unsigned)nchunk);
  colsum_partial<<<grid, 256, 0, stream>>>(x, ld, rows, F, rpc, ws);
  splitk_reduce_kernel<<<(unsigned)ceil_div64(F, 256), 256, 0, stream>>>(ws, nchunk, F, F, out, accumulate);
  TSGNN_CHECK_LAUNCH();
  return TSGNN_OK;
}

int tsgnn_wgrad_reduce_sets_blocks(const int64_t* desc) {
  ReducePlan p;
  return reduce_plan(desc, p) == TSGNN_OK ? (int)p.first_block[p.n] : TSGNN_EINVAL;
}

int tsgnn_wgrad_reduce_sets_f32(const int64_t* desc, float* normparts, float* step_state, tsgnn_stream_t stream) {
  ReducePlan p;
  const int rc = reduce_plan(desc, p);
  if (rc != TSGNN_OK) return rc;
  TSGNN_KNAME("tn_rows_reduce_multi");
  return reduce_launch(p, normparts, step_state, stream);
}

int tsgnn_wgrad_blocks_plan(int64_t rows, int K_in, int N, int64_t ldz, int64_t lddu, int* nslab, int64_t* rows_per_slab,
                            int64_t* ws_floats) {
  if (!nslab || !rows_per_slab || !ws_floats || rows < 0) return TSGNN_EINVAL;
  *nslab = 0; *rows_per_slab = 0; *ws_floats = 0;
  if (K_in <= 0 || N <= 0 || K_in > 512 || N > 512 || (ldz % 4) || (lddu % 4) || (N % 4)) return TSGNN_OK;
  const int nsets = ((K_in + 127) / 128) * ((N + 127) / 128);
  if (nsets > WB_MAXSETS) return TSGNN_OK;
  static const int per_cu = [] { const char* e = getenv("TSGNN_WGRAD_BLOCKS_PER_CU"); const int v = e ? atoi(e) : 2; return v > 0 ? v : 2; }();
  int64_t ns = (int64_t)per_cu * device_cu_count() / (2 * nsets);
  if (ns < 1) ns = 1;
  int64_t rps = ceil_div64(rows > 0 ? rows : 1, ns);
  rps = ((rps + 31) / 32) * 32;
  *rows_per_slab = rps;
  *nslab = (int)(rows > 0 ? ceil_div64(rows, rps) : 1);
  *ws_floats = (int64_t)nsets * (*nslab) * WB_SET_FLOATS;
  return TSGNN_OK;
}

static int wgrad_blocks_launch(const float* z, int64_t ldz, const float* du, int64_t lddu, int64_t rows, int K_in, int N, int nslab,
                               int64_t rows_per_slab, float* ws, float* dw, int64_t lddw, int oi, float* db, tsgnn_stream_t stream) {
  if (!z || !du || !ws || rows < 0 || nslab <= 0 || rows_per_slab <= 0 || K_in <= 0 || N <= 0 || (dw && lddw < (oi ? K_in : N))) return TSGNN_EINVAL;
  if (K_in > 512 || N > 512 || (ldz % 4) || (lddu % 4) || (N % 4) || ldz < ((K_in + 3) / 4) * 4 || lddu < N ||
      ((reinterpret_cast<uintptr_t>(z) | reinterpret_cast<uintptr_t>(du)) & 15))
    return TSGNN_EUNSUPPORTED;
// ... 33 lines not shown
```

two-stage-gnn_amd/csrc/optim.hip:

```cpp
#include "common.h"
#include "../../include/tsgnn.h"

namespace {

constexpr int NPART = 256;

__device__ __forceinline__ bool poisoned(const float* __restrict__ poison) {
  return poison != nullptr && __hip_atomic_load(poison, __ATOMIC_RELAXED, __HIP_MEMORY_SCOPE_AGENT) != 0.f;
}

__global__ __launch_bounds__(256) void sqnorm_partial(const float* __restrict__ g, int64_t n, float* __restrict__ part) {
  __shared__ float lds[4];
  float s = 0.f;
  for (int64_t i = (int64_t)blockIdx.x * 256 + threadIdx.x; i < n; i += (int64_t)gridDim.x * 256) s = fmaf(g[i], g[i], s);
  s = wave_sum(s);
  if ((threadIdx.x & 63) == 0) lds[threadIdx.x >> 6] = s;
  __syncthreads();
  if (threadIdx.x == 0) part[blockIdx.x] = lds[0] + lds[1] + lds[2] + lds[3];
}
__global__ __launch_bounds__(256) void sqnorm_final(const float* __restrict__ part, int nparts, float grad_scale, float max_norm,
                                                    float* __restrict__ state, const float* __restrict__ poison) {
  __shared__ float lds[4];
  if (poisoned(poison)) { if (threadIdx.x == 0) state[3] = 1.f; return; }
  float s = threadIdx.x < nparts ? part[threadIdx.x] : 0.f;
  s = wave_sum(s);
  if ((threadIdx.x & 63) == 0) lds[threadIdx.x >> 6] = s;
  __syncthreads();
  if (threadIdx.x == 0) {
    const float norm = sqrtf(lds[0] + lds[1] + lds[2] + lds[3]) * grad_scale;
    float coef = 1.f;
    if (max_norm > 0.f) coef = fminf(max_norm / (norm + 1e-6f), 1.f);
    state[0] += 1.f;
    state[1] = norm;
    state[2] = coef * grad_scale;
  }
}
__global__ void adam_update(float* __restrict__ p, const float* __restrict__ g, float* __restrict__ m, float* __restrict__ v,
                            int64_t n, float lr, float b1, float b2, float eps, float wd, const float* __restrict__ state,
                            const float* __restrict__ poison) {
  const int64_t i = (int64_t)blockIdx.x * blockDim.x + threadIdx.x;
  if (i >= n || poisoned(poison)) return;
  const float step = state[0], scale = state[2];
  const float bc1 = 1.f - powf(b1, step), bc2 = 1.f - powf(b2, step);
  float gi = g[i] * scale;
  if (wd != 0.f) gi = fmaf(wd, p[i], gi);
  const float mi = fmaf(b1, m[i], (1.f - b1) * gi);
  const float vi = fmaf(b2, v[i], (1.f - b2) * gi * gi);
  m[i] = mi; v[i] = vi;
  const float denom = sqrtf(vi) / sqrtf(bc2) + eps;
  p[i] -= (lr / bc1) * (mi / denom);
}


constexpr int CV = 4;
#ifndef TSGNN_SELFNORM_MAX_N
#define TSGNN_SELFNORM_MAX_N 131072
#endif
constexpr int64_t SELFNORM_MAX_N = TSGNN_SELFNORM_MAX_N;
__global__ __launch_bounds__(256) void clip_adam_selfnorm(float* __restrict__ p, const float* __restrict__ g, float* __restrict__ m,
                                                          float* __restrict__ v, int64_t n, float lr, float b1, float b2, float eps,
                                                          float wd, float max_norm, float grad_scale, float* __restrict__ state,
                                                          unsigned* __restrict__ done, const float* __restrict__ poison) {
  __shared__ float lds[4];
  const int tid = threadIdx.x;
  if (poisoned(poison)) {
    if (tid == 0) {
      const unsigned prev = __hip_atomic_fetch_add(done, 1u, __ATOMIC_ACQ_REL, __HIP_MEMORY_SCOPE_AGENT);
      if (prev == gridDim.x - 1) { __hip_atomic_store(done, 0u, __ATOMIC_RELAXED, __HIP_MEMORY_SCOPE_AGENT); state[3] = 1.f; }
    }
    return;
  }
  const int64_t base = ((int64_t)blockIdx.x * 256 + tid) * CV;
  float gv[CV], pv[CV], mv[CV], vv[CV];
#pragma unroll
  for (int c = 0; c < CV; ++c) {
    const bool ok = (base + c) < n;
    gv[c] = ok ? g[base + c] : 0.f; pv[c] = ok ? p[base + c] : 0.f; mv[c] = ok ? m[base + c] : 0.f; vv[c] = ok ? v[base + c] : 0.f;
  }
  const float step = state[0] + 1.f;
  const float4* __restrict__ g4 = reinterpret_cast<const float4*>(g);
  const int64_t n4 = n >> 2;
  float s0 = 0.f, s1 = 0.f, s2 = 0.f, s3 = 0.f;
  int64_t i = tid;
  for (; i + 15 * 256 < n4; i += 16 * 256) {
    float4 q[16];
#pragma unroll
    for (int u = 0; u < 16; ++u) q[u] = g4[i + u * 256];
#pragma unroll
    for (int u = 0; u < 16; u += 4) {
      s0 = fmaf(q[u].x, q[u].x, s0); s0 = fmaf(q[u].y, q[u].y, s0); s0 = fmaf(q[u].z, q[u].z, s0); s0 = fmaf(q[u].w, q[u].w, s0);
      s1 = fmaf(q[u + 1].x, q[u + 1].x, s1); s1 = fmaf(q[u + 1].y, q[u + 1].y, s1); s1 = fmaf(q[u + 1].z, q[u + 1].z, s1); s1 = fmaf(q[u + 1].w, q[u + 1].w, s1);
      s2 = fmaf(q[u + 2].x, q[u + 2].x, s2); s2 = fmaf(q[u + 2].y, q[u + 2].y, s2); s2 = fmaf(q[u + 2].z, q[u + 2].z, s2); s2 = fmaf(q[u + 2].w, q[u + 2].w, s2);
      s3 = fmaf(q[u + 3].x, q[u + 3].x, s3); s3 = fmaf(q[u + 3].y, q[u + 3].y, s3); s3 = fmaf(q[u + 3].z, q[u + 3].z, s3); s3 = fmaf(q[u + 3].w, q[u + 3].w, s3);
    }
  }
  for (; i + 3 * 256 < n4; i += 4 * 256) {
    const float4 a = g4[i], b = g4[i + 256], c = g4[i + 512], d = g4[i + 768];
    s0 = fmaf(a.x, a.x, s0); s0 = fmaf(a.y, a.y, s0); s0 = fmaf(a.z, a.z, s0); s0 = fmaf(a.w, a.w, s0);
    s1 = fmaf(b.x, b.x, s1); s1 = fmaf(b.y, b.y, s1); s1 = fmaf(b.z, b.z, s1); s1 = fmaf(b.w, b.w, s1);
    s2 = fmaf(c.x, c.x, s2); s2 = fmaf(c.y, c.y, s2); s2 = fmaf(c.z, c.z, s2); s2 = fmaf(c.w, c.w, s2);
    s3 = fmaf(d.x, d.x, s3); s3 = fmaf(d.y, d.y, s3); s3 = fmaf(d.z, d.z, s3); s3 = fmaf(d.w, d.w, s3);
  }
  for (; i < n4; i += 256) {
    const float4 a = g4[i];
    s0 = fmaf(a.x, a.x, s0); s0 = fmaf(a.y, a.y, s0); s0 = fmaf(a.z, a.z, s0); s0 = fmaf(a.w, a.w, s0);
  }
  for (int64_t k = (n4 << 2) + tid; k < n; k += 256) s1 = fmaf(g[k], g[k], s1);
  float s = wave_sum((s0 + s1) + (s2 + s3));
  if ((tid & 63) == 0) lds[tid >> 6] = s;
  __syncthreads();
  const float norm = sqrtf((lds[0] + lds[1]) + (lds[2] + lds[3])) * grad_scale;
  float coef = 1.f;
  if (max_norm > 0.f) coef = fminf(max_norm / (norm + 1e-6f), 1.f);
  const float scale = coef * grad_scale;
  const float bc1 = 1.f - powf(b1, step), bc2 = 1.f - powf(b2, step);
#pragma unroll
  for (int c = 0; c < CV; ++c) {
    const int64_t k = base + c;
    if (k < n) {
      float gi = gv[c] * scale;
      if (wd != 0.f) gi = fmaf(wd, pv[c], gi);
      const float mi = fmaf(b1, mv[c], (1.f - b1) * gi);
      const float vi = fmaf(b2, vv[c], (1.f - b2) * gi * gi);
      m[k] = mi; v[k] = vi;
      const float denom = sqrtf(vi) / sqrtf(bc2) + eps;
      p[k] = pv[c] - (lr / bc1) * (mi / denom);
    }
  }
  if (tid == 0) {
    const unsigned prev = __hip_atomic_fetch_add(done, 1u, __ATOMIC_ACQ_REL, __HIP_MEMORY_SCOPE_AGENT);
    if (prev == gridDim.x - 1) {
      __hip_atomic_store(done, 0u, __ATOMIC_RELAXED, __HIP_MEMORY_SCOPE_AGENT);
      state[0] = step; state[1] = norm; state[2] = scale;
    }
  }
}

__global__ __launch_bounds__(256) void adam_from_partials(float* __restrict__ p, const float* __restrict__ g, float* __restrict__ m,
                                                          float* __restrict__ v, int64_t n, float lr, float b1, float b2, float eps,
                                                          float wd, float max_norm, float* __restrict__ state,
                                                          const float* __restrict__ parts, int nparts, const float* __restrict__ poison) {
  __shared__ float lds[4];
  const int tid = threadIdx.x;
  if (poisoned(poison)) {
    if (blockIdx.x == 0 && tid == 0) { state[0] -= 1.f; state[3] = 1.f; }
    return;
  }
  const int64_t base = ((int64_t)blockIdx.x * 256 + tid) * CV;
  float gv[CV], pv[CV], mv[CV], vv[CV];
#pragma unroll
  for (int c = 0; c < CV; ++c) {
    const bool ok = (base + c) < n;
    gv[c] = ok ? g[base + c] : 0.f; pv[c] = ok ? p[base + c] : 0.f; mv[c] = ok ? m[base + c] : 0.f; vv[c] = ok ? v[base + c] : 0.f;
  }
  float t = 0.f;
  for (int k0 = tid; k0 < nparts; k0 += 4 * 256) {
    float q[4];
#pragma unroll
    for (int u = 0; u < 4; ++u) q[u] = parts[min(k0 + 256 * u, nparts - 1)];
#pragma unroll
    for (int u = 0; u < 4; ++u) if (k0 + 256 * u < nparts) t += q[u];
  }
  t = wave_sum(t);
  if ((tid & 63) == 0) lds[tid >> 6] = t;
  __syncthreads();
  const float norm = sqrtf((lds[0] + lds[1]) + (lds[2] + lds[3]));
  float coef = 1.f;
  if (max_norm > 0.f) coef = fminf(max_norm / (norm + 1e-6f), 1.f);
  const float step = state[0];
  if (blockIdx.x == 0 && tid == 0) { state[1] = norm; state[2] = coef; }
  const float bc1 = 1.f - powf(b1, step), bc2 = 1.f - powf(b2, step);
#pragma unroll
  for (int c = 0; c < CV; ++c) {
    const int64_t i = base + c;
    if (i < n) {
      float gi = gv[c] * coef;
      if (wd != 0.f) gi = fmaf(wd, pv[c], gi);
      const float mi = fmaf(b1, mv[c], (1.f - b1) * gi);
      const float vi = fmaf(b2, vv[c], (1.f - b2) * gi * gi);
      m[i] = mi; v[i] = vi;
      const float denom = sqrtf(vi) / sqrtf(bc2) + eps;
      p[i] = pv[c] - (lr / bc1) * (mi / denom);
    }
  }
}


__global__ __launch_bounds__(256) void softmax_ce_kernel(const float* __restrict__ logits, int64_t ld, const int64_t* __restrict__ label,
                                                         int B, int C, float* __restrict__ loss, float* __restrict__ dlogits) {
  __shared__ float lds[4];
  float part = 0.f;
  for (int b = threadIdx.x; b < B; b += 256) {
    const float* row = logits + (int64_t)b * ld;
    float m = -INFINITY;
    for (int c = 0; c < C; ++c) m = fmaxf(m, row[c]);
    float d = 0.f;
    for (int c = 0; c < C; ++c) d += expf(row[c] - m);
    const int y = (int)label[b];
    const float logz = m + logf(d);
    part += logz - row[y];
    const float invB = 1.f / (float)B;
    for (int c = 0; c < C; ++c) dlogits[(int64_t)b * C + c] = (expf(row[c] - logz) - (c == y ? 1.f : 0.f)) * invB;
  }
  part = wave_sum(part);
  if ((threadIdx.x & 63) == 0) lds[threadIdx.x >> 6] = part;
  __syncthreads();
  if (threadIdx.x == 0) *loss = ((lds[0] + lds[1]) + (lds[2] + lds[3])) / (float)B;
}

}

extern "C" {

int tsgnn_softmax_ce_f32(const float* logits, int64_t ld, const int64_t* label, int B, int C, float* loss, float* dlogits,
                         tsgnn_stream_t stream) {
  if (!logits || !label || !loss || !dlogits || B <= 0 || C <= 0 || ld < C) return TSGNN_EINVAL;
  TSGNN_KNAME("softmax_ce_kernel");
  softmax_ce_kernel<<<1, 256, 0, stream>>>(logits, ld, label, B, C, loss, dlogits);
  TSGNN_CHECK_LAUNCH();
  return TSGNN_OK;
}

int tsgnn_adam_from_partials_f32(float* param, const float* grad, float* m, float* v, int64_t n, float lr, float beta1, float beta2,
                                 float eps, float weight_decay, float max_norm, float* state, const float* parts, int nparts,
                                 const float* poison, tsgnn_stream_t stream) {
  if (!param || !grad || !m || !v || !state || !parts || n <= 0 || nparts <= 0) return TSGNN_EINVAL;
  TSGNN_KNAME("adam_from_partials");
  adam_from_partials<<<(unsigned)ceil_div64(n, 256 * CV), 256, 0, stream>>>(param, grad, m, v, n, lr, beta1, beta2, eps, weight_decay,
                                                                           max_norm, state, parts, nparts, poison);
  TSGNN_CHECK_LAUNCH();
  return TSGNN_OK;
}

int tsgnn_clip_adam_step_f32(float* param, const float* grad, float* m, float* v, int64_t n, float lr, float beta1,
                             float beta2, float eps, float weight_decay, float max_norm, float grad_scale, float* state,
                             float* ws, const float* poison, tsgnn_stream_t stream) {
  if (!param || !grad || !m || !v || !state || !ws || n <= 0) return TSGNN_EINVAL;
  if (reinterpret_cast<uintptr_t>(ws) & 7) return TSGNN_EINVAL;
  if (n <= SELFNORM_MAX_N) {
    const int nbc = (int)ceil_div64(n, 256 * CV);
    TSGNN_KNAME("clip_adam_selfnorm");
    clip_adam_selfnorm<<<nbc, 256, 0, stream>>>(param, grad, m, v, n, lr, beta1, beta2, eps, weight_decay, max_norm, grad_scale, state,
                                                reinterpret_cast<unsigned*>(ws + 256), poison);
    TSGNN_CHECK_LAUNCH();
    return TSGNN_OK;
  }
  int nb = (int)ceil_div64(n, 256 * 8);
  if (nb > NPART) nb = NPART;
  TSGNN_KNAME("sqnorm_partial + sqnorm_final + adam_update");
  sqnorm_partial<<<nb, 256, 0, stream>>>(grad, n, ws);
  sqnorm_final<<<1, 256, 0, stream>>>(ws, nb, grad_scale, max_norm, state, poison);
  adam_update<<<(unsigned)ceil_div64(n, 256), 256, 0, stream>>>(param, grad, m, v, n, lr, beta1, beta2, eps, weight_decay, state, poison);
  TSGNN_CHECK_LAUNCH();
  return TSGNN_OK;
}

}
```

two-stage-gnn_amd/data_parallel.py:

```python
import os

import torch
import torch.distributed as dist

from . import _native as nat
from . import message_passing as mp


class FlatTrainer:

    def __init__(self, model, lr=1e-3, betas=(0.9, 0.999), eps=1e-8, weight_decay=0.0, clip=2.0, group=None, direct_grads=True,
                 defer_loss=False, buckets=None):
        self.model = model
        self.buckets = int(os.environ.get("TSGNN_AR_BUCKETS", 1)) if buckets is None else int(buckets)
        self.defer_loss = bool(defer_loss)
        self.params = [p for p in model.parameters() if p.requires_grad]
        dev = self.params[0].device
        self.views = []
        self._pads = []
        off = 0
        for p in self.params:
            pad = (-off) % 4
            self._pads.append(pad)
            off += pad
            self.views.append((off, p.numel()))
            off += p.numel()
        self.numel = off
        self.flat_param = torch.zeros(self.numel, dtype=torch.float32, device=dev)
        self._grad_store = torch.zeros(self.numel + 4, dtype=torch.float32, device=dev)
        self.flat_grad = self._grad_store[:self.numel]
        self._err_slot = self._grad_store[self.numel:self.numel + 1]
        for p, (o, n) in zip(self.params, self.views):
            self.flat_param[o:o + n].copy_(p.data.reshape(-1))
            p.data = self.flat_param[o:o + n].view_as(p.data)
        self.lr, self.betas, self.eps, self.wd, self.clip = lr, betas, eps, weight_decay, clip
        self.on_gpu = dev.type == "cuda"
        self.exp_avg = torch.zeros_like(self.flat_param)
        self.exp_avg_sq = torch.zeros_like(self.flat_param)
        self.state = torch.zeros(4, dtype=torch.float32, device=dev)
        self.poison = mp.device_error_word(dev) if dev.type == "cuda" else None
        self.ws = torch.zeros(264, dtype=torch.float32, device=dev)
        self._zeros = [torch.zeros_like(p).reshape(-1) for p in self.params]
        self._pad_zeros = [torch.zeros(k, dtype=torch.float32, device=dev) if k else None for k in self._pads]
        self.group = group
        self.world = dist.get_world_size(group) if dist.is_available() and dist.is_initialized() else 1
        if self.world > 1:
            dist.broadcast(self.flat_param, src=dist.get_global_rank(group, 0) if group is not None else 0, group=group)
        self.sink = None
        self._dirty = set()
        if direct_grads and self.on_gpu:
            self.sink = mp.GradSink()
            for p, (o, n) in zip(self.params, self.views):
                self.sink.views[p.data_ptr()] = self.flat_grad[o:o + n].view_as(p.data)
            self.sink.norm_parts = torch.zeros(4096, dtype=torch.float32, device=dev)
            self.sink.step_state = self.state
        self.always_reduce = False
        self._early = None
        self._early_issued = False
        self._allow_early = True
        self._side = torch.cuda.Stream() if (self.on_gpu and self.buckets > 1) else None

    def _reducing(self):
        return (self.world > 1 or self.always_reduce) and dist.is_available() and dist.is_initialized()

    def _range_of(self, params):
        ptrs = {q.data_ptr() for q in params}
        idx = sorted(i for i, p in enumerate(self.params) if p.data_ptr() in ptrs)
        if not idx or idx != list(range(idx[0], idx[-1] + 1)):
            return None
        start = self.views[idx[0]][0] - self._pads[idx[0]]
        last = idx[-1]
        end = self.numel if last == len(self.params) - 1 else self.views[last + 1][0] - self._pads[last + 1]
        return start, end

    def _on_ready(self, params):
        if self._early_issued or not self._allow_early or self._side is None or not self._reducing():
            return
        rng = self._range_of([p for p in params if p is not None])
        if rng is None or rng[1] - rng[0] <= 0:
            return
        if self._early is None:
            self._early = rng
        elif rng != self._early:
            return
        self._side.wait_stream(torch.cuda.current_stream())
        with torch.cuda.stream(self._side):
            dist.all_reduce(self.flat_grad[rng[0]:rng[1]], op=dist.ReduceOp.SUM, group=self.group)
        self._early_issued = True

    def zero_grad(self):
        for p in self.params:
            p.grad = None
        self._norm_ready = False
        self._early_issued = False
        mp.CE_DEFER = self.defer_loss and self.on_gpu
        if self.sink is not None:
            self.sink.ready_cb = self._on_ready if (self._side is not None and self._reducing()) else None
            self.sink.written.clear()
            self.sink.reset_norm()
            self.sink.norm_enabled = self.world == 1 and not self.always_reduce
            mp.GRAD_SINK = self.sink

    def backward(self, loss):
        loss.backward(gradient=mp.unit_seed(loss.device) if loss.is_cuda and loss.dim() == 0 else None)

    def gather_grads(self):
        written = ()
        mp.CE_DEFER = False
        if self.sink is not None:
            mp.GRAD_SINK = None
            written = self.sink.written
            self._norm_ready = (bool(written) and self.sink.stepped and written == self.sink.normed and not self.sink.reused
                                and all(p.grad is None for p in self.params) and self.world == 1 and not self.always_reduce)
        if not written:
            parts = []
            for p, z, pz in zip(self.params, self._zeros, self._pad_zeros):
                if pz is not None:
                    parts.append(pz)
                parts.append(p.grad.reshape(-1) if p.grad is not None else z)
            torch.cat(parts, out=self.flat_grad)
            self._dirty = {i for i, p in enumerate(self.params) if p.grad is not None}
            return self.flat_grad
        cp_dst, cp_src, add_dst, add_src, zero_dst = [], [], [], [], []
        for i, (p, (o, n)) in enumerate(zip(self.params, self.views)):
            direct = p.data_ptr() in written
            if p.grad is not None:
                if direct and self._early_issued and self._early[0] <= o < self._early[1]:
                    extra = p.grad.reshape(-1).contiguous()
                    dist.all_reduce(extra, op=dist.ReduceOp.SUM, group=self.group)
                    torch.cuda.current_stream().wait_stream(self._side)
                    self.flat_grad[o:o + n].add_(extra)
                elif direct:
                    add_dst.append(self.flat_grad[o:o + n]); add_src.append(p.grad.reshape(-1))
                else:
                    cp_dst.append(self.flat_grad[o:o + n]); cp_src.append(p.grad.reshape(-1))
                self._dirty.add(i)
            elif direct:
                self._dirty.add(i)
            elif i in self._dirty:
                zero_dst.append(self.flat_grad[o:o + n])
                self._dirty.discard(i)
        if cp_dst:
            torch._foreach_copy_(cp_dst, cp_src)
        if add_dst:
            torch._foreach_add_(add_dst, add_src)
        if zero_dst:
            torch._foreach_zero_(zero_dst)
        return self.flat_grad

    def all_reduce(self):
        if self.world > 1 or self.always_reduce:
            if self.poison is not None:
                self._err_slot.copy_(self.poison)
            if self._early_issued:
                a, b = self._early
                for s_, e_ in ((0, a), (b, self.numel + 4)):
                    if e_ > s_:
                        dist.all_reduce(self._grad_store[s_:e_], op=dist.ReduceOp.SUM, group=self.group)
                torch.cuda.current_stream().wait_stream(self._side)
                return
            dist.all_reduce(self._grad_store, op=dist.ReduceOp.SUM, group=self.group)

    def _poison_word(self):
        return self._err_slot if ((self.world > 1 or self.always_reduce) and self.poison is not None) else self.poison

    def apply(self):
        scale = 1.0 / self.world
        if not self.on_gpu:
            raise RuntimeError("FlatTrainer.apply runs the HIP optimiser kernel; parameters must live on the GPU "
                               "(no CPU fallback)")
        if getattr(self, "_norm_ready", False):
            nat.call("adam_from_partials_f32", self.flat_param, self.flat_grad, self.exp_avg, self.exp_avg_sq, self.numel,
                     float(self.lr), float(self.betas[0]), float(self.betas[1]), float(self.eps), float(self.wd), float(self.clip),
                     self.state, self.sink.norm_parts, int(self.sink.norm_used), self._poison_word())
            return
        if self.sink is not None and self.sink.stepped:
            self.state[0] -= 1.0
        nat.call("clip_adam_step_f32", self.flat_param, self.flat_grad, self.exp_avg, self.exp_avg_sq, self.numel,
                 float(self.lr), float(self.betas[0]), float(self.betas[1]), float(self.eps), float(self.wd),
                 float(self.clip), float(scale), self.state, self.ws, self._poison_word())

    def check(self):
        torch.cuda.synchronize()
        skipped = self.on_gpu and float(self.state[3]) != 0.0
        try:
            mp.check_device_errors()
            if skipped and (self.world > 1 or self.always_reduce):
                raise RuntimeError("a bounded device-wide barrier timed out on another rank: every rank skipped the optimiser update "
                                   "since (the replicas still hold identical parameters)")
        finally:
            if skipped:
                self.state[3] = 0.0
                self._err_slot.zero_()
                torch.cuda.synchronize()

    def step(self, loss_fn):
        self.zero_grad()
        loss = loss_fn()
        self.backward(loss)
        self.gather_grads()
        self.all_reduce()
        self.apply()
        return loss


class _capture:

    def __init__(self, graph, **kw):
        self._ctx = torch.cuda.graph(graph, **kw)

    def __enter__(self):
        import gc
        self._was = gc.isenabled()
        gc.collect()
        gc.disable()
        try:
            return self._ctx.__enter__()
        except BaseException:
            if self._was:
                gc.enable()
            raise

    def __exit__(self, *exc):
        import gc
        try:
            return self._ctx.__exit__(*exc)
        finally:
            if self._was:
                gc.enable()


class GraphedStep:

    def __init__(self, trainer, loss_fn, warmup=3, use_graph=True, stream=None, steps_per_replay=1):
        self.trainer, self.loss_fn, self.use_graph = trainer, loss_fn, use_graph
        self.multi = trainer.world > 1 or trainer.always_reduce
        self.stream = stream if stream is not None else torch.cuda.Stream()
        self.loss = None
        self._fb = self._opt = None
        self._fbk, self.steps_per_replay = None, 1
        self.one_graph = False
        with torch.cuda.stream(self.stream):
            snap = [t.clone() for t in (trainer.flat_param, trainer.exp_avg, trainer.exp_avg_sq, trainer.state)] if warmup else None
            for _ in range(warmup):
                self._fwd_bwd(); trainer.all_reduce(); trainer.apply()
            if snap is not None:
                for t, s_ in zip((trainer.flat_param, trainer.exp_avg, trainer.exp_avg_sq, trainer.state), snap):
                    t.copy_(s_)
            torch.cuda.synchronize()
            mp.check_device_errors()
            if not use_graph:
                return
            if self.multi and dist.is_initialized():
                dist.barrier(group=trainer.group)
                torch.cuda.synchronize()
                if dist.get_backend(trainer.group) == "nccl":
                    import time
                    time.sleep(0.25)
            mode = {"capture_error_mode": "thread_local"} if self.multi else {}
            want = os.environ.get("TSGNN_GRAPH_ALLREDUCE", "auto") if self.multi else "0"
            self.mode_note = ""
            if want == "auto" and self.multi and dist.is_initialized() and dist.get_backend(trainer.group) != "nccl" \
                    and os.environ.get("TSGNN_ONE_GRAPH_ANY_BACKEND") != "1":
                want = "0"
            if self.multi and want != "0":
                self._snap = [t.clone() for t in self._bufs()]
                graph = self._capture_one(mode)
        if self.multi and want != "0":
            ok = self._try_one_graph(graph, verify=(want != "1"))
            graph = None
            if not ok:
                self._fb = None
                if want == "1":
                    raise RuntimeError("TSGNN_GRAPH_ALLREDUCE=1: the all-reduce could not be captured into the step's hipGraph "
                                       "on every rank; use TSGNN_GRAPH_ALLREDUCE=auto (checked, falls back) or 0 (two graphs)")
            self.one_graph = ok
        if self._fb is None:
            with torch.cuda.stream(self.stream):
                self._capture_two(mode)
        self._snap = None
        self._loss1 = self._lossk = self.loss
        if int(steps_per_replay) > 1 and not self.multi:
            self.steps_per_replay = int(steps_per_replay)
            with torch.cuda.stream(self.stream):
                snap = [t.clone() for t in (trainer.flat_param, trainer.exp_avg, trainer.exp_avg_sq, trainer.state)]
                self._fbk = torch.cuda.CUDAGraph()
                with _capture(self._fbk, stream=self.stream):
                    for _ in range(self.steps_per_replay):
                        self._fwd_bwd()
                        trainer.apply()
                for t, s_ in zip((trainer.flat_param, trainer.exp_avg, trainer.exp_avg_sq, trainer.state), snap):
                    t.copy_(s_)
                torch.cuda.synchronize()
            self._lossk, self.loss = self.loss, self._loss1

    def _bufs(self):
        tr = self.trainer
        return tr.flat_param, tr.exp_avg, tr.exp_avg_sq, tr.state

    def _agree(self, ok):
        tr = self.trainer
        if dist.is_initialized():
            with torch.cuda.stream(self.stream):
                flag = torch.tensor([1.0 if ok else 0.0], device=tr.flat_param.device)
                dist.all_reduce(flag, op=dist.ReduceOp.MIN, group=tr.group)
                ok = bool(flag.item() > 0.5)
                torch.cuda.synchronize()
        return ok

    def _capture_two(self, mode):
        trainer = self.trainer
        if self.multi and dist.is_initialized() and dist.get_backend(trainer.group) == "nccl":
            torch.cuda.synchronize()
            import time
            time.sleep(0.25)
        trainer._allow_early = not self.multi
        self._fb = torch.cuda.CUDAGraph()
        with _capture(self._fb, stream=self.stream, **mode):
            self._fwd_bwd()
            if not self.multi:
                trainer.apply()
        if self.multi:
            self._opt = torch.cuda.CUDAGraph()
            with _capture(self._opt, stream=self.stream, **mode):
                trainer.apply()

    def _abandon_stream(self):
        tr = self.trainer
        self.stream = torch.cuda.Stream()
        if tr._side is not None:
            tr._side = torch.cuda.Stream()
        tr._early_issued = False
        with torch.cuda.stream(self.stream):
            for _ in range(4):
                try:
                    torch.cuda.synchronize()
                    break
                except Exception:
                    pass
            for t, s_ in zip(self._bufs(), self._snap):
                t.copy_(s_)
            torch.cuda.synchronize()

    def _capture_one(self, mode):
        tr = self.trainer
        graph = torch.cuda.CUDAGraph()
        try:
            tr._allow_early = True
            with _capture(graph, stream=self.stream, **mode):
                self._fwd_bwd()
                if os.environ.get("TSGNN_TEST_BREAK_CAPTURE") in ("all", str(dist.get_rank() if dist.is_initialized() else 0)):
                    torch.cuda.current_stream().synchronize()
                tr.all_reduce()
                tr.apply()
        except Exception as e:
            print("GraphedStep: one-graph capture failed (%s: %s)" % (type(e).__name__, str(e).splitlines()[0]), flush=True)
            return None
        return graph

    def _try_one_graph(self, graph, verify):
        tr = self.trainer
        bufs, snap = self._bufs(), self._snap
        captured = graph is not None
        if not captured:
            self._abandon_stream()
        all_captured = self._agree(captured)
        if not all_captured:
            self.mode_note = " (one-graph step failed its capture on %s: fell back)" % ("this rank" if not captured else "another rank")
            return False
        ok = True
        with torch.cuda.stream(self.stream):
            if verify:
                graph.replay()
                torch.cuda.synchronize()
                got = tr.flat_param.clone()
                for t, s_ in zip(bufs, snap):
                    t.copy_(s_)
                self._fwd_bwd(); tr.all_reduce(); tr.apply()
                torch.cuda.synchronize()
                scale = float(tr.flat_param.abs().max()) + 1e-30
                ok = bool(torch.isfinite(got).all()) and float((got - tr.flat_param).abs().max()) <= 1e-5 * scale
            for t, s_ in zip(bufs, snap):
                t.copy_(s_)
            torch.cuda.synchronize()
        if verify:
            ok = self._agree(ok)
            if not ok:
                self.mode_note = " (one-graph step failed its check: fell back)"
        if ok:
            self._fb = graph
        return ok

    def describe(self):
        if not self.use_graph:
            return "eager"
        if not self.multi:
            k = ("; run(): %d consecutive steps per graph launch" % self.steps_per_replay) if self._fbk is not None else ""
            return "one graph: forward + backward + bucket + optimiser" + k
        bk = ", early bucket [%d, %d) all-reduced on a side branch" % self.trainer._early if self.trainer._early else ""
        if self.one_graph:
            return "one graph incl. the captured all-reduce" + bk
        return "two graphs around the eagerly issued all-reduce" + getattr(self, "mode_note", "")

    def _fwd_bwd(self):
        tr = self.trainer
        tr.zero_grad()
        self.loss = self.loss_fn()
        tr.backward(self.loss)
        tr.gather_grads()

    def synchronize(self):
        self.stream.synchronize()
        self.trainer.check()

    def loss_value(self):
        self.synchronize()
        return float(self.loss.detach())

    def run(self, n):
        n = int(n)
        self._since_check = getattr(self, "_since_check", 0) + n
        if self._fbk is not None:
            with torch.cuda.stream(self.stream):
                while n >= self.steps_per_replay:
                    self._fbk.replay()
                    n -= self.steps_per_replay
                    self.loss = self._lossk
        for _ in range(n):
            self.step()
        if self._since_check >= self.CHECK_EVERY:
            self._since_check = 0
            self.synchronize()
        return self.loss

    CHECK_EVERY = 4096

    def step(self):
        with torch.cuda.stream(self.stream):
            if not self.use_graph:
                self._fwd_bwd(); self.trainer.all_reduce(); self.trainer.apply()
            elif not self.multi or self.one_graph:
                self._fb.replay()
                self.loss = self._loss1
            else:
                self._fb.replay(); self.trainer.all_reduce(); self._opt.replay()
                self.loss = self._loss1
        return self.loss
```

two-stage-gnn_amd/message_passing.py:

```python
import os

import numpy as np
import torch

from . import _native as nat


def _f32(*shape, device, zero=False):
    return (torch.zeros if zero else torch.empty)(*shape, dtype=torch.float32, device=device)


def _check(x, rows=None):
    if not x.is_cuda:
        raise RuntimeError("two_stage_gnn_amd operators run on the GPU only (no CPU fallback)")
    if x.dtype != torch.float32 or x.dim() != 2:
        raise ValueError("expected a float32 [rows, features] matrix")
    if rows is not None and x.size(0) != rows:
        raise ValueError("feature matrix has %d rows, the graph batch has %d" % (x.size(0), rows))
    return x if x.is_contiguous() else x.contiguous()


def spmm_raw(rowptr, col, val, x, n_rows, self_w=None, self_scalar=0.0, relu_in=False, out=None, accumulate=False):
    y = out if out is not None else _f32(x.size(0), x.size(1), device=x.device)
    nat.call("csr_spmm_f32", rowptr, col, val, self_w, x, x.stride(0), y, y.stride(0), int(n_rows), int(x.size(1)),
             float(self_scalar), int(relu_in), int(accumulate))
    return y


ELL_MAX_ROWS = 16384


def ell_ok(x):
    F = x.size(1)
    return F % 4 == 0 and F <= 256 and x.stride(0) % 4 == 0 and x.data_ptr() % 16 == 0


def spmm_ell(g, x, self_scalar=0.0, out=None, rows=None):
    ell, W, tail = g.ell()
    y = out if out is not None else _f32(x.size(0), x.size(1), device=x.device)
    n = g.total_rows if rows is None else int(rows)
    nat.call("ell_spmm_f32", ell, W, x, x.stride(0), y, y.stride(0), n, int(x.size(1)), float(self_scalar))
    if tail is not None:
        spmm_raw(tail[0], tail[1], None, x, n, out=y, accumulate=True)
    return y


class _Aggregate(torch.autograd.Function):

    @staticmethod
    def forward(ctx, x, g, add_self, val, self_w):
        x = _check(x, g.total_rows)
        ctx.g, ctx.add_self, ctx.val, ctx.self_w = g, add_self, val, self_w
        ctx.x = x if ctx.needs_input_grad[3] or ctx.needs_input_grad[4] else None
        ctx.fast = val is None and self_w is None and g.val is None and ell_ok(x) and g.total_rows <= ELL_MAX_ROWS
        if ctx.fast:
            return spmm_ell(g, x, 1.0 if add_self else 0.0)
        return spmm_raw(g.rowptr, g.col, val, x, g.total_rows, self_w=self_w, self_scalar=1.0 if add_self else 0.0)

    @staticmethod
    def backward(ctx, dy):
        g = ctx.g
        dy = _check(dy)
        if ctx.fast and g.symmetric and ell_ok(dy):
            return spmm_ell(g, dy, 1.0 if ctx.add_self else 0.0), None, None, None, None
        val = ctx.val.detach() if ctx.val is not None else None
        self_w = ctx.self_w.detach() if ctx.self_w is not None else None
        rowptr_t, col_t, val_t = g.transposed(val)
        dx = spmm_raw(rowptr_t, col_t, val_t, dy, g.total_rows, self_w=self_w,
                      self_scalar=1.0 if ctx.add_self else 0.0)
        dval = dself = None
        if ctx.x is not None:
            if dy.size(1) > 1024:
                raise NotImplementedError("weight gradients of the aggregation for more than 1024 features")
            dval = _f32(max(g.nnz, 1), device=dy.device)
            dself = _f32(g.total_rows, device=dy.device)
            nat.call("sddmm_rows_f32", g.rowptr, g.col, dy, dy.stride(0), ctx.x, ctx.x.stride(0), g.total_rows, int(dy.size(1)),
                     dval, dself)
            dval = dval[: ctx.val.numel()] if ctx.needs_input_grad[3] else None
            dself = dself if ctx.needs_input_grad[4] else None
        return dx, None, None, dval, dself


def aggregate(x, g, add_self=False, val="graph", self_w=None):
    if isinstance(val, str):
        val = g.val
    return _Aggregate.apply(x, g, bool(add_self), val, self_w)


def gemm(A, sam, sak, B, sbk, sbn, C, scm, scn, M, N, K, batch=1, stride_a=0, stride_b=0, stride_c=0,
         seg_ptr=None, ragged=0, max_seg=0, alpha=1.0, accumulate=False):
    nat.call("gemm_f32", A, int(sam), int(sak), B, int(sbk), int(sbn), C, int(scm), int(scn), int(M), int(N), int(K),
             int(batch), int(stride_a), int(stride_b), int(stride_c), seg_ptr, int(ragged), int(max_seg), float(alpha),
             int(accumulate))


def gemm_tn_splitk(Z, K_in, dU, out=None):
    R, N = dU.size(0), dU.size(1)
    plan = np.zeros(1, dtype=np.int32)
    need = np.zeros(1, dtype=np.int64)
    nat.call_nostream("gemm_splitk_plan", int(K_in), int(N), int(R), plan.ctypes.data, need.ctypes.data)
    ws = _f32(max(int(need[0]), 1), device=dU.device)
    out = out if out is not None else _f32(K_in, N, device=dU.device)
    nat.call("gemm_splitk_f32", Z, 1, Z.stride(0), dU, dU.stride(0), 1, out, int(K_in), int(N), int(R), int(plan[0]),
             ws, 0)
    return out


def wgrad_plan(rows, K_in, N, ldz, lddu, blocked=False):
    nslab = np.zeros(1, dtype=np.int32)
    rps = np.zeros(1, dtype=np.int64)
    need = np.zeros(1, dtype=np.int64)
    nat.call_nostream("wgrad_blocks_plan" if blocked else "linear_wgrad_plan", int(rows), int(K_in), int(N), int(ldz), int(lddu),
                      nslab.ctypes.data, rps.ctypes.data, need.ctypes.data)
    return int(nslab[0]), int(rps[0]), int(need[0])


def linear_wgrad_slabs(z, K_in, du, bias_only_rows=0):
    R, N = du.size(0) - int(bias_only_rows), du.size(1)
    nslab, rps, need = wgrad_plan(R, K_in, N, z.stride(0), du.stride(0))
    if nslab <= 0 or z.data_ptr() % 16 or du.data_ptr() % 16:
        return None
    ws = _f32(need, device=du.device)
    nat.call("linear_wgrad_f32", z, z.stride(0), du, du.stride(0), R, int(K_in), int(N), nslab, rps, int(bias_only_rows), ws, None, None)
    return ws, nslab


def wgrad_set(ws, nslab, K, N, dw, db=None, n_db=None, tail=None, kn=0, lddw=None, blocked=False):
    if lddw is None:
        lddw = dw.stride(0) if dw is not None else 0
    return (ws, int(nslab), int(K), int(N), dw, int(lddw), db, int(N if n_db is None else n_db), tail, int(kn), int(bool(blocked)))


def _desc(sets):
    words = [len(sets)]
    for st in sets:
        words += [0 if v is None else (v.data_ptr() if torch.is_tensor(v) else int(v)) for v in st]
    return np.asarray(words, dtype=np.int64)


def _norm_args(norm_sink, d):
    if norm_sink is None:
        return None, None
    nblk = int(nat.lib().tsgnn_wgrad_reduce_sets_blocks(d.ctypes.data))
    if nblk < 0:
        raise RuntimeError("wgrad_reduce: invalid slab set")
    parts = norm_sink.norm_slots(nblk)
    if parts is None or norm_sink.stepped:
        return parts, None
    norm_sink.stepped = True
    return parts, norm_sink.step_state


REDUCE_SETS = 12


def wgrad_reduce(sets, norm_sink=None):
    if nat._defer is not None:
        raise RuntimeError("wgrad_reduce cannot be recorded under nat.deferred()")
    normed = norm_sink is not None
    for i in range(0, len(sets), REDUCE_SETS):
        d = _desc(sets[i:i + REDUCE_SETS])
        parts, step = _norm_args(norm_sink, d)
        normed = normed and parts is not None
        nat.call("wgrad_reduce_sets_f32", d.ctypes.data, parts, step)
    return normed


def wgrad_reduce_multi(sets, norm_sink=None):
    normed = norm_sink is not None
    for i in range(0, len(sets), 4):
        chunk = list(sets[i:i + 4])
        parts, step = (_norm_args(norm_sink, _desc([wgrad_set(*st, kn=1, lddw=st[3]) for st in chunk]))
                       if norm_sink is not None else (None, None))
        normed = normed and parts is not None
        args = []
        for ws, nslab, K, N, dw, db in chunk + [(None, 0, 0, 0, None, None)] * (4 - len(chunk)):
            args += [ws, int(nslab), int(K), int(N), dw, db]
        nat.call("wgrad_reduce_multi_f32", *args, parts, step)
    return normed


class WgradSets:

    def __init__(self, launcher=wgrad_reduce, max_sets_with_shares=None):
        self.launcher, self.max_sets = launcher, max_sets_with_shares
        self.sink = GRAD_SINK
        self.sets, self.params, self.sunk, self.all_sunk = [], [], [], True

    def grad(self, param, shape):
        if param is None:
            return None
        self.params.append(param)
        v = self.sink.take(param, shape) if self.sink is not None else None
        if v is None:
            self.all_sunk = False
            return _f32(*shape, device=param.device)
        self.sunk.append(v)
        return v

    def autograd_grad(self, buf):
        return None if any(buf is v for v in self.sunk) else buf

    def add(self, record):
        self.sets.append(record)

    def close(self):
        if not self.sets:
            return
        shares = (self.sink is not None and len(self.params) > 0 and self.all_sunk
                  and (self.max_sets is None or len(self.sets) <= self.max_sets))
        if self.launcher(self.sets, norm_sink=self.sink if shares else None):
            self.sink.normed.update(p.data_ptr() for p in self.params)
        self.sets = []


def linear_wgrad_oi(z, K_in, du, want_db):
    R, N = int(du.size(0)), int(du.size(1))
    nslab, rps, need = wgrad_plan(R, K_in, N, z.stride(0), du.stride(0), blocked=True)
    if nslab <= 0 or z.data_ptr() % 16 or du.data_ptr() % 16 or z.stride(0) < (int(K_in) + 3) // 4 * 4:
        return None
    ws = _f32(need, device=du.device)
    dw = _f32(N, int(K_in), device=du.device)
    db = _f32(N, device=du.device) if want_db else None
    if not nat.try_call("wgrad_blocks_oi_f32", z, z.stride(0), du, du.stride(0), R, int(K_in), N, nslab, rps, ws, dw, dw.stride(0), db):
        return None
    return dw, db


def linear_wgrad(z, K_in, du, want_db, du_job=None):
    R, N = du.size(0), du.size(1)
    nslab, rps, need = wgrad_plan(R, K_in, N, z.stride(0), du.stride(0))
    if du_job is not None:
        part, nb, F_du, dws, dbs = du_job
        if nslab > 0 and nb <= 256 and z.data_ptr() % 16 == 0 and du.data_ptr() % 16 == 0:
            ws = _f32(need, device=du.device)
            dw = _f32(K_in, N, device=du.device)
            db = _f32(N, device=du.device) if want_db else None
            nat.call("linear_wgrad_du_f32", z, z.stride(0), du, du.stride(0), R, int(K_in), int(N), nslab, rps, ws, dw, db, part, int(nb),
                     int(F_du), dws, dbs)
            return dw, db
        nat.call("sag_du_reduce_f32", part, int(nb), int(F_du), dws, dbs)
    if nslab > 0 and z.data_ptr() % 16 == 0 and du.data_ptr() % 16 == 0:
        ws = _f32(need, device=du.device)
        dw = _f32(K_in, N, device=du.device)
        db = _f32(N, device=du.device) if want_db else None
        nat.call("linear_wgrad_f32", z, z.stride(0), du, du.stride(0), R, int(K_in), int(N), nslab, rps, 0, ws, dw, db)
        return dw, db
    if z.data_ptr() % 16 == 0 and du.data_ptr() % 16 == 0 and z.stride(0) % 4 == 0 and du.stride(0) % 4 == 0:
        if K_in > 128 and N <= 128 and N % 4 == 0 and K_in % 4 == 0 and K_in <= 512:
            dw = _f32(K_in, N, device=du.device)
            db = _f32(N, device=du.device) if want_db else None
            sets = []
            for k0 in range(0, K_in, 128):
                kc = min(128, K_in - k0)
                got = linear_wgrad_slabs(z[:, k0:], kc, du)
                if got is None:
                    sets = None
                    break
                sets.append((got[0], got[1], kc, N, dw[k0:k0 + kc], db if k0 == 0 else None))
            if sets:
                wgrad_reduce_multi(sets)
                return dw, db
        elif N > 128 and K_in <= 128 and K_in % 4 == 0 and N % 4 == 0 and N <= 512 and z.size(1) >= K_in:
            dwt = _f32(N, K_in, device=du.device)
            sets = []
            for n0 in range(0, N, 128):
                nc = min(128, N - n0)
                got = linear_wgrad_slabs(du[:, n0:], nc, z[:, :K_in] if z.size(1) != K_in else z)
                if got is None:
                    sets = None
                    break
                sets.append((got[0], got[1], nc, K_in, dwt[n0:n0 + nc], None))
            if sets:
                wgrad_reduce_multi(sets)
                return dwt.t(), (colsum(du) if want_db else None)
    if K_in <= 4:
        need = np.zeros(1, dtype=np.int64)
        nat.call_nostream("wgrad_narrow_plan", int(R), int(K_in), int(N), need.ctypes.data)
        ws = _f32(max(int(need[0]), 1), device=du.device)
        dwb = _f32(K_in + 1, N, device=du.device)
        nat.call("wgrad_narrow_f32", z, z.stride(0), du, du.stride(0), int(R), int(K_in), int(N), ws, dwb)
        return dwb[:K_in], (dwb[K_in] if want_db else None)
    return gemm_tn_splitk(z, K_in, du), (colsum(du) if want_db else None)


def colsum(x):
    R, F = x.size(0), x.size(1)
    out = _f32(F, device=x.device)
    ws = _f32(max(1, (R + 127) // 128) * F, device=x.device)
    nat.call("colsum_f32", x, x.stride(0), int(R), int(F), out, ws, 0)
    return out


def rowgemm_ok(a, lda, b, ldb, K, N, trans_b):
    return bool(nat.lib().tsgnn_rowgemm_supported(a.data_ptr(), int(lda), b.data_ptr(), int(ldb), None, 0, int(K), int(N),
                                                  int(trans_b)))


class _LinearL2Norm(torch.autograd.Function):

    @staticmethod
    def forward(ctx, z, weight, bias, normalize):
        z = _check(z)
        w = weight.contiguous()
        K, N = w.size(0), w.size(1)
        if z.size(1) < K:
            raise ValueError("input has %d features, weight expects %d" % (z.size(1), K))
        R = z.size(0)
        v = _f32(R, N, device=z.device)
        rinv = _f32(R, device=z.device) if normalize else None
        if rowgemm_ok(z, z.stride(0), w, w.stride(0), K, N, False):
            nat.call("rowgemm_f32", z, z.stride(0), w, w.stride(0), 0, bias, v, v.stride(0), rinv, R, K, N, int(normalize), 0)
        else:
            nat.call("linear_l2norm_f32", z, z.stride(0), w, w.stride(0), bias, v, v.stride(0), rinv, R, K, N,
                     int(normalize))
        ctx.save_for_backward(z, w, v if normalize else None, rinv)
        ctx.has_bias = bias is not None
        ctx.normalize = normalize
        return v

    @staticmethod
    def backward(ctx, dv):
        z, w, v, rinv = ctx.saved_tensors
        dv = _check(dv)
        R, N, K = dv.size(0), w.size(1), w.size(0)
        if ctx.normalize:
            du = torch.empty_like(dv)
            nat.call("l2norm_bwd_f32", v, v.stride(0), dv, dv.stride(0), rinv, du, du.stride(0), R, N)
        else:
            du = dv
        dz = dw = db = None
        if ctx.needs_input_grad[0]:
            ldz = z.size(1)
            dz = _f32(R, ldz, device=dv.device, zero=(ldz > K))
            if rowgemm_ok(du, du.stride(0), w, w.stride(0), N, K, True):
                nat.call("rowgemm_f32", du, du.stride(0), w, w.stride(0), 1, None, dz, dz.stride(0), None, R, N, K, 0, 0)
            else:
                gemm(du, du.stride(0), 1, w, 1, w.stride(0), dz, dz.stride(0), 1, R, K, N)
        want_db = ctx.has_bias and ctx.needs_input_grad[2]
        if ctx.needs_input_grad[1]:
            dw, db = linear_wgrad(z, K, du, want_db)
        elif want_db:
            db = colsum(du)
        return dz, dw, db, None


def linear_l2norm(z, weight, bias=None, normalize=True):
    return _LinearL2Norm.apply(z, weight, bias, bool(normalize))


class _LinearOI(torch.autograd.Function):

    @staticmethod
    def forward(ctx, x, weight, bias):
        x = _check(x)
        w = weight.contiguous()
        N, K = w.size(0), w.size(1)
        R = x.size(0)
        y = _f32(R, N, device=x.device)
        if rowgemm_ok(x, x.stride(0), w, w.stride(0), K, N, True):
            nat.call("rowgemm_f32", x, x.stride(0), w, w.stride(0), 1, bias, y, y.stride(0), None, R, K, N, 0, 0)
        else:
            gemm(x, x.stride(0), 1, w, 1, w.stride(0), y, y.stride(0), 1, R, N, K)
# ... 399 lines not shown

    @staticmethod
    def backward(ctx, dout, _darg, dpass=None):
        (arg,) = ctx.saved_tensors
        if dout is None:
            return dpass, None, None, None, None
        return readout_bwd_raw(dout, arg, ctx.g, ctx.rows, ctx.ghost_unused, dpass), None, None, None, None


def readout_max(x, g, return_arg=False, into=None):
    out, arg = _ReadoutMax.apply(x, g, False, False, into)
    return (out, arg) if return_arg else out


def readout_max_pass(x, g, ghost_unused=False, into=None):
    out, _arg, xp = _ReadoutMax.apply(x, g, True, bool(ghost_unused), into)
    return out, xp


class _Into:
    __slots__ = ("t",)

    def __init__(self, t):
        self.t = t


class _JoinColumns(torch.autograd.Function):
    @staticmethod
    def forward(ctx, cols, *parts):
        ctx.widths = [p.size(1) for p in parts]
        return cols.buf

    @staticmethod
    def backward(ctx, d):
        out, c0 = [None], 0
        for w in ctx.widths:
            out.append(d[:, c0:c0 + w])
            c0 += w
        return tuple(out)


class ReadoutColumns:

    def __init__(self, B, total, device):
        self.buf = _f32(int(B), int(total), device=device)
        self.c0, self.parts = 0, 0

    def take(self, F):
        F = int(F)
        if self.c0 < 0 or self.c0 + F > self.buf.size(1) or F % 4 or self.c0 % 4:
            self.c0 = -1
            return None
        t = torch.empty(0, dtype=torch.float32, device=self.buf.device)
        t.set_(self.buf.untyped_storage(), self.buf.storage_offset() + self.c0, (self.buf.size(0), F), (self.buf.stride(0), 1))
        self.c0 += F
        self.parts += 1
        return _Into(t)

    def join(self, parts):
        if self.c0 == self.buf.size(1) and self.parts == len(parts):
            return _JoinColumns.apply(self, *parts)
        return torch.cat(parts, dim=1)


class _PackRows(torch.autograd.Function):
    @staticmethod
    def forward(ctx, xp, g, ld):
        if not xp.is_cuda:
            raise RuntimeError("two_stage_gnn_amd operators run on the GPU only (no CPU fallback)")
        xp = xp.contiguous().float()
        B, nmax, F = xp.shape
        if B != g.B or nmax != g.nmax:
            raise ValueError("padded features [%d,%d,*] do not match the graph batch [%d,%d]" % (B, nmax, g.B, g.nmax))
        out = _f32(g.total_rows, ld, device=xp.device, zero=True)
        nat.call("pack_rows_f32", xp, nmax, F, g.row_graph, g.row_slot, g.n_rows, out, out.stride(0))
        ctx.g, ctx.F = g, F
        return out

    @staticmethod
    def backward(ctx, dout):
        g = ctx.g
        dout = _check(dout)
        dxp = _f32(g.B, g.nmax, ctx.F, device=dout.device)
        nat.call("unpack_rows_f32", g.graph_ptr, g.B, g.nmax, g.n_rows, 0, dout, dout.stride(0), ctx.F, 0.0, dxp)
        return dxp, None, None


def pack_rows(x_padded, g, ld=None):
    F = x_padded.size(2)
    if g.layout == "padded":
        if ld not in (None, F):
            raise ValueError("padded layout keeps the feature width")
        x = x_padded.contiguous().float().reshape(g.B * g.nmax, F)
        return x
    return _PackRows.apply(x_padded, g, F if ld is None else int(ld))


class _UnpackRows(torch.autograd.Function):
    @staticmethod
    def forward(ctx, x, g, fill):
        x = _check(x, g.total_rows)
        F = x.size(1)
        out = _f32(g.B, g.nmax, F, device=x.device)
        nat.call("unpack_rows_f32", g.graph_ptr, g.B, g.nmax, g.n_rows, g.n_ghost, x, x.stride(0), F, float(fill), out)
        ctx.g, ctx.F = g, F
        return out

    @staticmethod
    def backward(ctx, dout):
        g = ctx.g
        dout = dout.contiguous()
        dx = _f32(g.total_rows, ctx.F, device=dout.device, zero=True)
        nat.call("pack_rows_f32", dout, g.nmax, ctx.F, g.row_graph, g.row_slot, g.n_rows, dx, dx.stride(0))
        if g.n_ghost:
            nat.call("unpack_rows_bwd_ghost_f32", g.graph_ptr, g.B, g.nmax, g.n_rows, dout, ctx.F, dx, dx.stride(0))
        return dx, None, None


def unpack_rows(x, g, fill=0.0):
    if g.layout == "padded":
        return x.reshape(g.B, g.nmax, x.size(1))
    return _UnpackRows.apply(x, g, fill)


class _MaskGhost(torch.autograd.Function):

    @staticmethod
    def forward(ctx, x, n_real):
        y = x.clone()
        y[n_real:].zero_()
        ctx.n_real = n_real
        return y

    @staticmethod
    def backward(ctx, dy):
        d = dy.clone()
        d[ctx.n_real:].zero_()
        return d, None


def mask_ghost_rows(x, g):
    return _MaskGhost.apply(x, g.n_rows) if g.n_ghost else x


class GradSink:

    def __init__(self):
        self.views = {}
        self.written = set()
        self.norm_parts = None
        self.step_state = None
        self.norm_enabled = False
        self.ready_cb = None
        self.reset_norm()

    def ready(self, params):
        if self.ready_cb is not None:
            self.ready_cb(params)

    def reset_norm(self):
        self.norm_used = 0
        self.normed = set()
        self.stepped = False
        self.reused = False

    def norm_slots(self, n):
        if not self.norm_enabled or self.norm_parts is None or self.norm_used + n > self.norm_parts.numel():
            return None
        v = self.norm_parts[self.norm_used:self.norm_used + n]
        self.norm_used += n
        return v

    def take(self, param, shape):
        key = param.data_ptr()
        v = self.views.get(key)
        if v is None or tuple(v.shape) != tuple(shape):
            return None
        if key in self.written:
            self.reused = True
            return None
        self.written.add(key)
        return v


DEVICE_ERRORS = []
_err_words = {}


def _dev_key(device):
    device = torch.device(device)
    if device.type == "cuda" and device.index is None:
        device = torch.device("cuda", torch.cuda.current_device())
    return device


def device_error_word(device):
    device = _dev_key(device)
    w = _err_words.get(device)
    if w is None:
        flag = torch.zeros(1, dtype=torch.float32, device=device)
        w = _err_words[device] = (flag, [])
        DEVICE_ERRORS.append((flag, "a bounded device-wide barrier timed out on %s (a kernel's workgroups were not all resident): the "
                                    "results of that launch are invalid; the optimiser skipped every update since" % (device,), w[1]))
    return w[0]


def register_barrier_words(device, words):
    device_error_word(device)
    _err_words[_dev_key(device)][1].append(words)


_clear_on_error = {}


def register_clear_on_error(t):
    import weakref
    lst = _clear_on_error.setdefault(_dev_key(t.device), [])
    lst.append(weakref.ref(t))
    if len(lst) > 4096:
        lst[:] = [r for r in lst if r() is not None]
    return t


def check_device_errors(synchronize=True):
    for flag, msg, state in DEVICE_ERRORS:
        if float(flag.item()) != 0.0:
            flag.zero_()
            for t in (state if isinstance(state, list) else [state]):
                if t is not None:
                    t.zero_()
            for ref in _clear_on_error.get(_dev_key(flag.device), []):
                t = ref()
                if t is not None:
                    t.zero_()
            raise RuntimeError(msg)


GRAD_SINK = None
_unit = {}


def _sink_or_new(param, shape, device):
    v = GRAD_SINK.take(param, shape) if (GRAD_SINK is not None and param is not None) else None
    if v is not None:
        return v, True
    return _f32(*shape, device=device), False


def unit_seed(device):
    device = torch.device(device)
    if device.type == "cuda" and device.index is None:
        device = torch.device("cuda", torch.cuda.current_device())
    t = _unit.get(device)
    if t is None:
        t = _unit[device] = torch.ones((), dtype=torch.float32, device=device)
    return t


HEAD_TAIL = os.environ.get("TSGNN_HEAD_TAIL", "1") != "0"
CE_DEFER = False
_deferred_ce = None


class _SoftmaxCE(torch.autograd.Function):

    @staticmethod
    def forward(ctx, logits, label, defer=False):
        B, C = logits.shape
        ctx.deferred = bool(defer and logits.is_contiguous() and logits.dtype == torch.float32)
        loss = _f32(1, device=logits.device)
        if ctx.deferred:
            ctx.loss = loss
            ctx.save_for_backward(logits, label.contiguous())
            return loss[0]
        logits = logits.contiguous().float()
        dlogits = _f32(B, C, device=logits.device)
        nat.call("softmax_ce_f32", logits, logits.stride(0), label.contiguous(), B, C, loss, dlogits)
        ctx.save_for_backward(dlogits)
        return loss[0]

    @staticmethod
    def backward(ctx, g):
        global _deferred_ce
        if ctx.deferred:
            logits, label = ctx.saved_tensors
            if g is _unit.get(g.device):
                ph = torch.empty_like(logits)
                _deferred_ce = (ph, logits, label, ctx.loss)
                return ph, None, None
            B, C = logits.shape
            dlogits = _f32(B, C, device=logits.device)
            nat.call("softmax_ce_f32", logits, logits.stride(0), label, B, C, ctx.loss, dlogits)
            return dlogits * g, None, None
        (dlogits,) = ctx.saved_tensors
        if g is _unit.get(g.device):
            return dlogits, None, None
        return dlogits * g, None, None


def take_deferred_ce(dy):
    global _deferred_ce
    d = _deferred_ce
    if d is not None and dy is d[0]:
        _deferred_ce = None
        return d[1], d[2], d[3]
    return None


def cross_entropy(logits, label):
    if logits.is_cuda and label.dtype == torch.int64:
        return _SoftmaxCE.apply(logits, label, bool(CE_DEFER and getattr(logits, "_tsgnn_defer_ce", False)))
    return torch.nn.functional.cross_entropy(logits, label, reduction="mean")


class _Head2(torch.autograd.Function):

    @staticmethod
# ... 137 lines not shown
```

Baseline: 258,400.

## Fuse final weight-gradient reduction with Adam step in one grid-synced launch

Defers the last wgrad slab reduction of backward and runs it together with the clipped Adam update in a single persistent kernel that uses a grid barrier between the reduction and the optimiser phases. This removes one kernel launch and the gap between the reduction and adam_from_partials. It also moves the barrier helpers into a shared header and adds give-up marking to the spin. The cost is added complexity, deferred state that must be flushed on every other path, and a dependence on all blocks being co-resident.

```diff
diff --git a/include/tsgnn.h b/include/tsgnn.h
--- a/include/tsgnn.h
+++ b/include/tsgnn.h
@@ -217,6 +217,12 @@
 int tsgnn_adam_from_partials_f32(float* param, const float* grad, float* m, float* v, int64_t n, float lr, float beta1, float beta2,
                                  float eps, float weight_decay, float max_norm, float* state, const float* parts, int nparts,
                                  const float* poison, tsgnn_stream_t stream);
+int tsgnn_wgrad_reduce_adam_f32(const float* ws0, int nslab0, int K0, int N0, float* dw0, float* db0, const float* ws1, int nslab1,
+                                int K1, int N1, float* dw1, float* db1, const float* ws2, int nslab2, int K2, int N2, float* dw2,
+                                float* db2, const float* ws3, int nslab3, int K3, int N3, float* dw3, float* db3,
+                                float* normparts, int part_first, int nparts, int bump_step, float* param, float* grad, float* m,
+                                float* v, int64_t n, float lr, float beta1, float beta2, float eps, float weight_decay, float max_norm,
+                                float* state, unsigned* sync, float* err, int max_resident, tsgnn_stream_t stream);
 int tsgnn_clip_adam_step_f32(float* param, const float* grad, float* m, float* v, int64_t n, float lr, float beta1,
                              float beta2, float eps, float weight_decay, float max_norm, float grad_scale, float* state,
                              float* ws, const float* poison, tsgnn_stream_t stream);
diff --git a/two-stage-gnn_amd/csrc/dense_stack.hip b/two-stage-gnn_amd/csrc/dense_stack.hip
--- a/two-stage-gnn_amd/csrc/dense_stack.hip
+++ b/two-stage-gnn_amd/csrc/dense_stack.hip
@@ -1,4 +1,5 @@
 #include "common.h"
+#include "grid_barrier.h"
 #include <utility>
 #include "../../include/tsgnn.h"
 
@@ -48,50 +49,6 @@
   unsigned* sync; float* err;
 };
 
-__device__ __forceinline__ void drain_stores() { asm volatile("s_waitcnt vmcnt(0)" ::: "memory"); }
-template <bool LIGHT = false>
-__device__ __forceinline__ void grid_barrier(unsigned* words, int& k, unsigned nblocks, float* err) {
-  drain_stores();
-  __syncthreads();
-  if (threadIdx.x == 0) {
-    if (LIGHT) __hip_atomic_fetch_add(words + k, 1u, __ATOMIC_RELAXED, __HIP_MEMORY_SCOPE_AGENT);
-    else __hip_atomic_fetch_add(words + k, 1u, __ATOMIC_RELEASE, __HIP_MEMORY_SCOPE_AGENT);
-    bool ok = false;
-    for (int spin = 0; spin < (1 << 21); ++spin) {
-      if (__hip_atomic_load(words + k, __ATOMIC_RELAXED, __HIP_MEMORY_SCOPE_AGENT) >= nblocks) { ok = true; break; }
-      __builtin_amdgcn_s_sleep(2);
-    }
-    if (!LIGHT) __builtin_amdgcn_fence(__ATOMIC_ACQUIRE, "agent");
-    if (!ok) __hip_atomic_store(err, 1.0f, __ATOMIC_RELAXED, __HIP_MEMORY_SCOPE_AGENT);
-    if (k > 0 && blockIdx.x == 0) __hip_atomic_store(words + k - 1, 0u, __ATOMIC_RELAXED, __HIP_MEMORY_SCOPE_AGENT);
-  }
-  ++k;
-  __syncthreads();
-}
-template <bool LIGHT = false>
-__device__ __forceinline__ void grid_arrive(unsigned* words, int k) {
-  drain_stores();
-  __syncthreads();
-  if (threadIdx.x == 0) {
-    if (LIGHT) __hip_atomic_fetch_add(words + k, 1u, __ATOMIC_RELAXED, __HIP_MEMORY_SCOPE_AGENT);
-    else __hip_atomic_fetch_add(words + k, 1u, __ATOMIC_RELEASE, __HIP_MEMORY_SCOPE_AGENT);
-  }
-}
-template <bool LIGHT = false>
-__device__ __forceinline__ void grid_wait(unsigned* words, int& k, unsigned nblocks, float* err) {
-  if (threadIdx.x == 0) {
-    bool ok = false;
-    for (int spin = 0; spin < (1 << 21); ++spin) {
-      if (__hip_atomic_load(words + k, __ATOMIC_RELAXED, __HIP_MEMORY_SCOPE_AGENT) >= nblocks) { ok = true; break; }
-      __builtin_amdgcn_s_sleep(2);
-    }
-    if (!LIGHT) __builtin_amdgcn_fence(__ATOMIC_ACQUIRE, "agent");
-    if (!ok) __hip_atomic_store(err, 1.0f, __ATOMIC_RELAXED, __HIP_MEMORY_SCOPE_AGENT);
-    if (k > 0 && blockIdx.x == 0) __hip_atomic_store(words + k - 1, 0u, __ATOMIC_RELAXED, __HIP_MEMORY_SCOPE_AGENT);
-  }
-  ++k;
-  __syncthreads();
-}
 __device__ __forceinline__ void group_barrier(unsigned* word, unsigned target, float* err) {
   drain_stores();
   __syncthreads();
@@ -114,15 +71,6 @@
 __device__ __forceinline__ float2 ds_get2(const float* p) {
   const unsigned long long bits = __hip_atomic_load(reinterpret_cast<const unsigned long long*>(p), __ATOMIC_RELAXED, __HIP_MEMORY_SCOPE_AGENT);
   return make_float2(__uint_as_float((unsigned)(bits & 0xffffffffull)), __uint_as_float((unsigned)(bits >> 32)));
-}
-__device__ __forceinline__ void grid_finish(unsigned* words, int k, unsigned nblocks) {
-  if (threadIdx.x == 0 && k > 0) {
-    const unsigned prev = __hip_atomic_fetch_add(words + 31, 1u, __ATOMIC_ACQ_REL, __HIP_MEMORY_SCOPE_AGENT);
-    if (prev == nblocks - 1) {
-      __hip_atomic_store(words + k - 1, 0u, __ATOMIC_RELAXED, __HIP_MEMORY_SCOPE_AGENT);
-      __hip_atomic_store(words + 31, 0u, __ATOMIC_RELAXED, __HIP_MEMORY_SCOPE_AGENT);
-    }
-  }
 }
 
 struct FastDiv {
diff --git a/two-stage-gnn_amd/csrc/gemm.hip b/two-stage-gnn_amd/csrc/gemm.hip
--- a/two-stage-gnn_amd/csrc/gemm.hip
+++ b/two-stage-gnn_amd/csrc/gemm.hip
@@ -1,4 +1,5 @@
 #include "common.h"
+#include "reduce_sets.h"
 #include <algorithm>
 #include <cstdlib>
 #include <type_traits>
@@ -210,27 +211,6 @@
   tn_rows_body<MT, NTt, NY>(g, tn_smem, blockIdx.x, blockIdx.y, gridDim.x);
 }
 
-__device__ __forceinline__ float slab_sum(const float* __restrict__ slabs, int nslab, int64_t per_slab, int64_t e, bool ok,
-                                          float (*lds)[64]) {
-  const int e_l = threadIdx.x & 63, grp = threadIdx.x >> 6;
-  float a0 = 0.f, a1 = 0.f, a2 = 0.f, a3 = 0.f;
-  if (ok) {
-    const int per = (nslab + 3) / 4;
-    const int s0 = grp * per, s1 = min(nslab, s0 + per);
-    int s = s0;
-    for (; s + 4 <= s1; s += 4) {
-      a0 += slabs[(int64_t)s * per_slab + e];
-      a1 += slabs[(int64_t)(s + 1) * per_slab + e];
-      a2 += slabs[(int64_t)(s + 2) * per_slab + e];
-      a3 += slabs[(int64_t)(s + 3) * per_slab + e];
-    }
-    for (; s < s1; ++s) a0 += slabs[(int64_t)s * per_slab + e];
-  }
-  lds[grp][e_l] = (a0 + a1) + (a2 + a3);
-  __syncthreads();
-  return (lds[0][e_l] + lds[1][e_l]) + (lds[2][e_l] + lds[3][e_l]);
-}
-
 __global__ __launch_bounds__(256) void tn_rows_reduce(const float* __restrict__ slabs, int64_t per_slab, int64_t n_w, float* __restrict__ out,
                                                       const int* __restrict__ seg_slab_ptr) {
   __shared__ float lds[4][64];
@@ -255,14 +235,6 @@
     else if (db) db[e - n_w] = v;
   }
 }
-
-struct ReduceSet {
-  const float* ws; int nslab, K, N;
-  float* dw; int64_t lddw; int kn;
-  float* db; int n_db; float* tail;
-};
-constexpr int RM_SETS = 12;
-struct ReduceMulti { int first_block[RM_SETS]; ReduceSet s[RM_SETS]; int n; float* normparts; float* step_state; };
 
 __global__ __launch_bounds__(256) void tn_rows_reduce_multi(ReduceMulti m) {
   __shared__ float lds[4][64];
@@ -297,7 +269,6 @@
 }
 }
 
-constexpr int RS_WORDS = 11;
 struct ReducePlan { ReduceSet s[RM_SETS * WB_MAXSETS]; int64_t first_block[RM_SETS * WB_MAXSETS + 1]; int n; };
 
 static int reduce_plan(const int64_t* desc, ReducePlan& p) {
@@ -362,6 +333,35 @@
   return rc != TSGNN_OK ? rc : reduce_launch(p, nullptr, nullptr, stream);
 }
 
+namespace tsgnn_detail {
+int reduce_positional_desc(const float* const* ws, const int* nslab, const int* K, const int* N, float* const* dw, float* const* db,
+                           int64_t* desc) {
+  std::fill(desc, desc + 1 + 4 * RS_WORDS, (int64_t)0);
+  for (int t = 0; t < 4; ++t) {
+    if (!ws[t]) continue;
+    if (K[t] <= 0) return TSGNN_EINVAL;
+    const int64_t r[RS_WORDS] = {(int64_t)(uintptr_t)ws[t], nslab[t], K[t], N[t], (int64_t)(uintptr_t)dw[t], N[t], (int64_t)(uintptr_t)db[t],
+                                 N[t], 0, 1, 0};
+    std::copy(r, r + RS_WORDS, desc + 1 + RS_WORDS * desc[0]++);
+  }
+  return TSGNN_OK;
+}
+int reduce_plan_one_launch(const int64_t* desc, ReduceMulti* m, int* nblocks) {
+  ReducePlan p;
+  const int rc = reduce_plan(desc, p);
+  if (rc != TSGNN_OK) return rc;
+  if (p.n < 1 || p.n > RM_SETS || p.first_block[p.n] > INT32_MAX) return TSGNN_EUNSUPPORTED;
+  *m = ReduceMulti{};
+  m->n = p.n;
+  for (int t = 0; t < p.n; ++t) {
+    m->s[t] = p.s[t];
+    m->first_block[t] = (int)p.first_block[t];
+  }
+  *nblocks = (int)p.first_block[p.n];
+  return TSGNN_OK;
+}
+}
+
 extern "C" {
 
 int tsgnn_gemm_f32(const float* A, int64_t sam, int64_t sak, const float* B, int64_t sbk, int64_t sbn, float* C,
@@ -436,14 +436,9 @@
   const int ns[4] = {nslab0, nslab1, nslab2, nslab3}, Ks[4] = {K0, K1, K2, K3}, Ns[4] = {N0, N1, N2, N3};
   float* dws[4] = {dw0, dw1, dw2, dw3};
   float* dbs[4] = {db0, db1, db2, db3};
-  int64_t desc[1 + 4 * RS_WORDS] = {0};
-  for (int t = 0; t < 4; ++t) {
-    if (!ws[t]) continue;
-    if (Ks[t] <= 0) return TSGNN_EINVAL;
-    const int64_t r[RS_WORDS] = {(int64_t)(uintptr_t)ws[t], ns[t], Ks[t], Ns[t], (int64_t)(uintptr_t)dws[t], Ns[t], (int64_t)(uintptr_t)dbs[t],
-                                 Ns[t], 0, 1, 0};
-    std::copy(r, r + RS_WORDS, desc + 1 + RS_WORDS * desc[0]++);
-  }
+  int64_t desc[1 + 4 * RS_WORDS];
+  const int rc = tsgnn_detail::reduce_positional_desc(ws, ns, Ks, Ns, dws, dbs, desc);
+  if (rc != TSGNN_OK) return rc;
   return tsgnn_wgrad_reduce_sets_f32(desc, normparts, step_state, stream);
 }
 
diff --git a/two-stage-gnn_amd/csrc/grid_barrier.h b/two-stage-gnn_amd/csrc/grid_barrier.h
--- /dev/null
+++ b/two-stage-gnn_amd/csrc/grid_barrier.h
@@ -0,0 +1,75 @@
+#pragma once
+#include "common.h"
+
+constexpr unsigned GRID_GAVE_UP = 0x40000000u;
+
+__device__ __forceinline__ void drain_stores() { asm volatile("s_waitcnt vmcnt(0)" ::: "memory"); }
+
+__device__ __forceinline__ bool grid_spin(unsigned* words, int k, unsigned nblocks, float* err) {
+  unsigned seen = 0;
+  for (int spin = 0; spin < (1 << 21); ++spin) {
+    seen = __hip_atomic_load(words + k, __ATOMIC_RELAXED, __HIP_MEMORY_SCOPE_AGENT);
+    if (seen >= nblocks) break;
+    __builtin_amdgcn_s_sleep(2);
+  }
+  for (int tries = 0; seen < nblocks && tries < 64; ++tries) {
+    unsigned want = seen;
+    if (__hip_atomic_compare_exchange_strong(words + k, &want, seen | GRID_GAVE_UP, __ATOMIC_RELAXED, __ATOMIC_RELAXED, __HIP_MEMORY_SCOPE_AGENT))
+      seen |= GRID_GAVE_UP;
+    else
+      seen = want;
+  }
+  const bool ok = seen >= nblocks && !(seen & GRID_GAVE_UP);
+  if (!ok) __hip_atomic_store(err, 1.0f, __ATOMIC_RELAXED, __HIP_MEMORY_SCOPE_AGENT);
+  return ok;
+}
+
+template <bool LIGHT = false>
+__device__ __forceinline__ void grid_arrive_one(unsigned* words, int k) {
+  if (LIGHT) __hip_atomic_fetch_add(words + k, 1u, __ATOMIC_RELAXED, __HIP_MEMORY_SCOPE_AGENT);
+  else __hip_atomic_fetch_add(words + k, 1u, __ATOMIC_RELEASE, __HIP_MEMORY_SCOPE_AGENT);
+}
+
+template <bool LIGHT = false>
+__device__ __forceinline__ bool grid_barrier(unsigned* words, int& k, unsigned nblocks, float* err, int* verdict = nullptr) {
+  bool ok = true;
+  drain_stores();
+  __syncthreads();
+  if (threadIdx.x == 0) {
+    grid_arrive_one<LIGHT>(words, k);
+    ok = grid_spin(words, k, nblocks, err);
+    if (!LIGHT) __builtin_amdgcn_fence(__ATOMIC_ACQUIRE, "agent");
+    if (k > 0 && blockIdx.x == 0) __hip_atomic_store(words + k - 1, 0u, __ATOMIC_RELAXED, __HIP_MEMORY_SCOPE_AGENT);
+    if (verdict) *verdict = ok ? 1 : 0;
+  }
+  ++k;
+  __syncthreads();
+  return ok;
+}
+template <bool LIGHT = false>
+__device__ __forceinline__ void grid_arrive(unsigned* words, int k) {
+  drain_stores();
+  __syncthreads();
+  if (threadIdx.x == 0) grid_arrive_one<LIGHT>(words, k);
+}
+template <bool LIGHT = false>
+__device__ __forceinline__ bool grid_wait(unsigned* words, int& k, unsigned nblocks, float* err) {
+  bool ok = true;
+  if (threadIdx.x == 0) {
+    ok = grid_spin(words, k, nblocks, err);
+    if (!LIGHT) __builtin_amdgcn_fence(__ATOMIC_ACQUIRE, "agent");
+    if (k > 0 && blockIdx.x == 0) __hip_atomic_store(words + k - 1, 0u, __ATOMIC_RELAXED, __HIP_MEMORY_SCOPE_AGENT);
+  }
+  ++k;
+  __syncthreads();
+  return ok;
+}
+__device__ __forceinline__ void grid_finish(unsigned* words, int k, unsigned nblocks) {
+  if (threadIdx.x == 0 && k > 0) {
+    const unsigned prev = __hip_atomic_fetch_add(words + 31, 1u, __ATOMIC_ACQ_REL, __HIP_MEMORY_SCOPE_AGENT);
+    if (prev == nblocks - 1) {
+      __hip_atomic_store(words + k - 1, 0u, __ATOMIC_RELAXED, __HIP_MEMORY_SCOPE_AGENT);
+      __hip_atomic_store(words + 31, 0u, __ATOMIC_RELAXED, __HIP_MEMORY_SCOPE_AGENT);
+    }
+  }
+}
diff --git a/two-stage-gnn_amd/csrc/optim.hip b/two-stage-gnn_amd/csrc/optim.hip
--- a/two-stage-gnn_amd/csrc/optim.hip
+++ b/two-stage-gnn_amd/csrc/optim.hip
@@ -1,5 +1,8 @@
 #include "common.h"
+#include "grid_barrier.h"
+#include "reduce_sets.h"
 #include "../../include/tsgnn.h"
+#include <algorithm>
 
 namespace {
 
@@ -136,39 +139,35 @@
   }
 }
 
-__global__ __launch_bounds__(256) void adam_from_partials(float* __restrict__ p, const float* __restrict__ g, float* __restrict__ m,
-                                                          float* __restrict__ v, int64_t n, float lr, float b1, float b2, float eps,
-                                                          float wd, float max_norm, float* __restrict__ state,
-                                                          const float* __restrict__ parts, int nparts, const float* __restrict__ poison) {
-  __shared__ float lds[4];
-  const int tid = threadIdx.x;
-  if (poisoned(poison)) {
-    if (blockIdx.x == 0 && tid == 0) { state[0] -= 1.f; state[3] = 1.f; }
-    return;
-  }
-  const int64_t base = ((int64_t)blockIdx.x * 256 + tid) * CV;
-  float gv[CV], pv[CV], mv[CV], vv[CV];
-#pragma unroll
-  for (int c = 0; c < CV; ++c) {
-    const bool ok = (base + c) < n;
-    gv[c] = ok ? g[base + c] : 0.f; pv[c] = ok ? p[base + c] : 0.f; mv[c] = ok ? m[base + c] : 0.f; vv[c] = ok ? v[base + c] : 0.f;
-  }
+
+template <bool ATOMIC>
+__device__ __forceinline__ float shares_partial(const float* __restrict__ parts, int nparts, int tid) {
   float t = 0.f;
   for (int k0 = tid; k0 < nparts; k0 += 4 * 256) {
     float q[4];
 #pragma unroll
-    for (int u = 0; u < 4; ++u) q[u] = parts[min(k0 + 256 * u, nparts - 1)];
+    for (int u = 0; u < 4; ++u) {
+      const float* src = parts + min(k0 + 256 * u, nparts - 1);
+      q[u] = ATOMIC ? __hip_atomic_load(src, __ATOMIC_RELAXED, __HIP_MEMORY_SCOPE_AGENT) : *src;
+    }
 #pragma unroll
     for (int u = 0; u < 4; ++u) if (k0 + 256 * u < nparts) t += q[u];
   }
+  return t;
+}
+__device__ __forceinline__ float norm_and_coef(float t, float max_norm, float* lds, float& coef) {
+  const int tid = threadIdx.x;
   t = wave_sum(t);
   if ((tid & 63) == 0) lds[tid >> 6] = t;
   __syncthreads();
   const float norm = sqrtf((lds[0] + lds[1]) + (lds[2] + lds[3]));
-  float coef = 1.f;
+  coef = 1.f;
   if (max_norm > 0.f) coef = fminf(max_norm / (norm + 1e-6f), 1.f);
-  const float step = state[0];
-  if (blockIdx.x == 0 && tid == 0) { state[1] = norm; state[2] = coef; }
+  return norm;
+}
+__device__ __forceinline__ void clip_adam_cv(float* __restrict__ p, float* __restrict__ m, float* __restrict__ v, int64_t n, int64_t base,
+                                             const float (&gv)[CV], const float (&pv)[CV], const float (&mv)[CV], const float (&vv)[CV],
+                                             float coef, float step, float lr, float b1, float b2, float eps, float wd) {
   const float bc1 = 1.f - powf(b1, step), bc2 = 1.f - powf(b2, step);
 #pragma unroll
   for (int c = 0; c < CV; ++c) {
@@ -183,6 +182,113 @@
       p[i] = pv[c] - (lr / bc1) * (mi / denom);
     }
   }
+}
+
+__global__ __launch_bounds__(256) void adam_from_partials(float* __restrict__ p, const float* __restrict__ g, float* __restrict__ m,
+                                                          float* __restrict__ v, int64_t n, float lr, float b1, float b2, float eps,
+                                                          float wd, float max_norm, float* __restrict__ state,
+                                                          const float* __restrict__ parts, int nparts, const float* __restrict__ poison) {
+  __shared__ float lds[4];
+  const int tid = threadIdx.x;
+  const float bad = poison ? __hip_atomic_load(poison, __ATOMIC_RELAXED, __HIP_MEMORY_SCOPE_AGENT) : 0.f;
+  const float step = state[0];
+  const int64_t base = ((int64_t)blockIdx.x * 256 + tid) * CV;
+  float gv[CV], pv[CV], mv[CV], vv[CV];
+#pragma unroll
+  for (int c = 0; c < CV; ++c) {
+    const int64_t i = min(base + c, n - 1);
+    gv[c] = g[i]; pv[c] = p[i]; mv[c] = m[i]; vv[c] = v[i];
+  }
+  const float t = shares_partial<false>(parts, nparts, tid);
+  if (bad != 0.f) {
+    if (blockIdx.x == 0 && tid == 0) { state[0] = step - 1.f; state[3] = 1.f; }
+    return;
+  }
+  float coef;
+  const float norm = norm_and_coef(t, max_norm, lds, coef);
+  if (blockIdx.x == 0 && tid == 0) { state[1] = norm; state[2] = coef; }
+  clip_adam_cv(p, m, v, n, base, gv, pv, mv, vv, coef, step, lr, b1, b2, eps, wd);
+}
+
+struct CloseArgs {
+  ReduceMulti r;
+  int rblocks;
+  int ablocks;
+  float* p; const float* g; float* m; float* v; int64_t n;
+  float lr, b1, b2, eps, wd, max_norm;
+  float* state; const float* parts; int nparts; int bump;
+  unsigned* sync; float* err;
+};
+__global__ __launch_bounds__(256) void tn_reduce_clip_adam(CloseArgs a) {
+  __shared__ float lds[4];
+  __shared__ int s_ok;
+  const int tid = threadIdx.x, e_l = tid & 63;
+  TR(0);
+  const float bad0 = __hip_atomic_load(a.err, __ATOMIC_RELAXED, __HIP_MEMORY_SCOPE_AGENT);
+  const float step0 = a.state[0];
+  const int64_t base = ((int64_t)blockIdx.x * 256 + tid) * CV;
+  float gv[CV], pv[CV], mv[CV], vv[CV];
+#pragma unroll
+  for (int c = 0; c < CV; ++c) {
+    const int64_t i = min(base + c, a.n - 1);
+    pv[c] = a.p[i]; mv[c] = a.m[i]; vv[c] = a.v[i];
+  }
+  const int ob = (int)blockIdx.x * 4 + __builtin_amdgcn_readfirstlane(tid >> 6);
+  if (ob < a.rblocks) {
+    int si = 0;
+#pragma unroll
+    for (int t = 1; t < RM_SETS; ++t) if (t < a.r.n && ob >= a.r.first_block[t]) si = t;
+    const ReduceSet& r = a.r.s[si];
+    const int64_t per_slab = (int64_t)(r.K + 1) * r.N;
+    const int64_t e = (int64_t)(ob - a.r.first_block[si]) * 64 + e_l;
+    float sq = 0.f;
+    if (e < per_slab) {
+      const float val = slab_sum_lane(r.ws, r.nslab, per_slab, e);
+      const int k = (int)e / r.N, nn = (int)e % r.N;
+      float* dst = nullptr;
+      if (k < r.K) dst = r.dw + (r.kn ? (int64_t)k * r.lddw + nn : (int64_t)nn * r.lddw + k);
+      else if (r.db && nn < r.n_db) dst = r.db + nn;
+      else if (r.tail && nn == r.n_db) dst = r.tail;
+      else if (r.K == 0 && r.dw && nn >= r.lddw && nn < r.lddw + r.n_db) dst = r.dw + (nn - r.lddw);
+      if (dst) { __hip_atomic_store(dst, val, __ATOMIC_RELAXED, __HIP_MEMORY_SCOPE_AGENT); sq = val * val; }
+    }
+    sq = wave_sum(sq);
+    if (e_l == 0) __hip_atomic_store(a.r.normparts + ob, sq, __ATOMIC_RELAXED, __HIP_MEMORY_SCOPE_AGENT);
+  }
+  TR(1);
+  int bar = 0;
+  grid_barrier<true>(a.sync, bar, gridDim.x, a.err, &s_ok);
+  TR(2);
+  const bool skip = bad0 != 0.f || s_ok == 0;
+#pragma unroll
+  for (int c = 0; c < CV; ++c) gv[c] = __hip_atomic_load(a.g + min(base + c, a.n - 1), __ATOMIC_RELAXED, __HIP_MEMORY_SCOPE_AGENT);
+  const float t = shares_partial<true>(a.parts, a.nparts, tid);
+  float coef;
+  const float norm = norm_and_coef(t, a.max_norm, lds, coef);
+  const float step = step0 + (float)a.bump;
+  TR_AFTER(__float_as_int(norm), 3);
+  if (!skip && (int)blockIdx.x < a.ablocks) clip_adam_cv(a.p, a.m, a.v, a.n, base, gv, pv, mv, vv, coef, step, a.lr, a.b1, a.b2, a.eps, a.wd);
+  if (blockIdx.x == 0 && tid == 0) {
+    if (skip) { a.state[0] = step0 - (float)(1 - a.bump); a.state[3] = 1.f; }
+    else { a.state[0] = step; a.state[1] = norm; a.state[2] = coef; }
+  }
+  grid_finish(a.sync, bar, gridDim.x);
+  TR(4);
+  TR_END();
+}
+
+int close_max_resident() {
+  constexpr int MAXDEV = 64;
+  static int cache[MAXDEV];
+  int dev = -1;
+  if (hipGetDevice(&dev) != hipSuccess || dev < 0 || dev >= MAXDEV) { (void)hipGetLastError(); return 0; }
+  if (cache[dev] != 0) return cache[dev] > 0 ? cache[dev] : 0;
+  int cus = 0, occ = 0;
+  bool ok = hipDeviceGetAttribute(&cus, hipDeviceAttributeMultiprocessorCount, dev) == hipSuccess;
+  ok = ok && hipOccupancyMaxActiveBlocksPerMultiprocessor(&occ, tn_reduce_clip_adam, 256, 0) == hipSuccess;
+  if (!ok) (void)hipGetLastError();
+  cache[dev] = (ok && cus > 0 && occ > 0) ? cus * occ : -1;
+  return cache[dev] > 0 ? cache[dev] : 0;
 }
 
 
@@ -232,6 +338,50 @@
   return TSGNN_OK;
 }
 
+int tsgnn_wgrad_reduce_adam_f32(const float* ws0, int nslab0, int K0, int N0, float* dw0, float* db0, const float* ws1, int nslab1,
+                                int K1, int N1, float* dw1, float* db1, const float* ws2, int nslab2, int K2, int N2, float* dw2,
+                                float* db2, const float* ws3, int nslab3, int K3, int N3, float* dw3, float* db3,
+                                float* normparts, int part_first, int nparts, int bump_step, float* param, float* grad, float* m,
+                                float* v, int64_t n, float lr, float beta1, float beta2, float eps, float weight_decay, float max_norm,
+                                float* state, unsigned* sync, float* err, int max_resident, tsgnn_stream_t stream) {
+  if (!param || !grad || !m || !v || !state || !normparts || !sync || !err || n <= 0 || nparts <= 0 || part_first < 0 ||
+      max_resident < 0 || (bump_step != 0 && bump_step != 1) || (reinterpret_cast<uintptr_t>(sync) & 3))
+    return TSGNN_EINVAL;
+  const float* ws[4] = {ws0, ws1, ws2, ws3};
+  const int ns[4] = {nslab0, nslab1, nslab2, nslab3}, Ks[4] = {K0, K1, K2, K3}, Ns[4] = {N0, N1, N2, N3};
+  float* dws[4] = {dw0, dw1, dw2, dw3};
+  float* dbs[4] = {db0, db1, db2, db3};
+  int64_t desc[1 + 4 * RS_WORDS];
+  int rc = tsgnn_detail::reduce_positional_desc(ws, ns, Ks, Ns, dws, dbs, desc);
+  if (rc != TSGNN_OK) return rc;
+  if (desc[0] == 0) return TSGNN_EINVAL;
+  CloseArgs a{};
+  rc = tsgnn_detail::reduce_plan_one_launch(desc, &a.r, &a.rblocks);
+  if (rc != TSGNN_OK) return rc;
+  if ((int64_t)part_first + a.rblocks > nparts) return TSGNN_EINVAL;
+  for (int t = 0; t < a.r.n; ++t) {
+    const ReduceSet& r = a.r.s[t];
+    float* const dst[3] = {r.dw, r.db, r.tail};
+    for (float* d : dst)
+      if (d && (d < grad || d >= grad + n)) return TSGNN_EINVAL;
+  }
+  const int64_t ablocks = ceil_div64(n, 256 * CV);
+  const int64_t grid = std::max<int64_t>(ceil_div64(a.rblocks, 4), ablocks);
+  int cap = close_max_resident();
+  if (max_resident > 0 && max_resident < cap) cap = max_resident;
+  if (grid > cap) return TSGNN_EUNSUPPORTED;
+  a.r.normparts = normparts + part_first;
+  a.ablocks = (int)ablocks;
+  a.p = param; a.g = grad; a.m = m; a.v = v; a.n = n;
+  a.lr = lr; a.b1 = beta1; a.b2 = beta2; a.eps = eps; a.wd = weight_decay; a.max_norm = max_norm;
+  a.state = state; a.parts = normparts; a.nparts = nparts; a.bump = bump_step;
+  a.sync = sync; a.err = err;
+  TSGNN_KNAME("tn_reduce_clip_adam");
+  tn_reduce_clip_adam<<<(unsigned)grid, 256, 0, stream>>>(a);
+  TSGNN_CHECK_LAUNCH();
+  return TSGNN_OK;
+}
+
 int tsgnn_clip_adam_step_f32(float* param, const float* grad, float* m, float* v, int64_t n, float lr, float beta1,
                              float beta2, float eps, float weight_decay, float max_norm, float grad_scale, float* state,
                              float* ws, const float* poison, tsgnn_stream_t stream) {
diff --git a/two-stage-gnn_amd/csrc/reduce_sets.h b/two-stage-gnn_amd/csrc/reduce_sets.h
--- /dev/null
+++ b/two-stage-gnn_amd/csrc/reduce_sets.h
@@ -0,0 +1,65 @@
+#pragma once
+#include "common.h"
+
+__device__ __forceinline__ float slab_sum(const float* __restrict__ slabs, int nslab, int64_t per_slab, int64_t e, bool ok,
+                                          float (*lds)[64]) {
+  const int e_l = threadIdx.x & 63, grp = threadIdx.x >> 6;
+  float a0 = 0.f, a1 = 0.f, a2 = 0.f, a3 = 0.f;
+  if (ok) {
+    const int per = (nslab + 3) / 4;
+    const int s0 = grp * per, s1 = min(nslab, s0 + per);
+    int s = s0;
+    for (; s + 4 <= s1; s += 4) {
+      a0 += slabs[(int64_t)s * per_slab + e];
+      a1 += slabs[(int64_t)(s + 1) * per_slab + e];
+      a2 += slabs[(int64_t)(s + 2) * per_slab + e];
+      a3 += slabs[(int64_t)(s + 3) * per_slab + e];
+    }
+    for (; s < s1; ++s) a0 += slabs[(int64_t)s * per_slab + e];
+  }
+  lds[grp][e_l] = (a0 + a1) + (a2 + a3);
+  __syncthreads();
+  return (lds[0][e_l] + lds[1][e_l]) + (lds[2][e_l] + lds[3][e_l]);
+}
+
+__device__ __forceinline__ float slab_sum_lane(const float* __restrict__ slabs, int nslab, int64_t per_slab, int64_t e) {
+  const int per = (nslab + 3) / 4;
+  float grp[4];
+#pragma unroll
+  for (int q = 0; q < 4; ++q) {
+    float a0 = 0.f, a1 = 0.f, a2 = 0.f, a3 = 0.f;
+    const int s0 = q * per, s1 = min(nslab, s0 + per);
+    const float* __restrict__ p = slabs + (int64_t)s0 * per_slab + e;
+    int s = s0;
+    for (; s + 16 <= s1; s += 16, p += 16 * per_slab) {
+      float v[16];
+#pragma unroll
+      for (int u = 0; u < 16; ++u) v[u] = p[(int64_t)u * per_slab];
+#pragma unroll
+      for (int u = 0; u < 16; u += 4) { a0 += v[u]; a1 += v[u + 1]; a2 += v[u + 2]; a3 += v[u + 3]; }
+    }
+    for (; s + 4 <= s1; s += 4, p += 4 * per_slab) {
+      const float v0 = p[0], v1 = p[per_slab], v2 = p[2 * per_slab], v3 = p[3 * per_slab];
+      a0 += v0; a1 += v1; a2 += v2; a3 += v3;
+    }
+    for (; s < s1; ++s, p += per_slab) a0 += p[0];
+    grp[q] = (a0 + a1) + (a2 + a3);
+  }
+  return (grp[0] + grp[1]) + (grp[2] + grp[3]);
+}
+
+struct ReduceSet {
+  const float* ws; int nslab, K, N;
+  float* dw; int64_t lddw; int kn;
+  float* db; int n_db; float* tail;
+};
+constexpr int RM_SETS = 12;
+struct ReduceMulti { int first_block[RM_SETS]; ReduceSet s[RM_SETS]; int n; float* normparts; float* step_state; };
+
+constexpr int RS_WORDS = 11;
+
+namespace tsgnn_detail {
+int reduce_positional_desc(const float* const* ws, const int* nslab, const int* K, const int* N, float* const* dw, float* const* db,
+                           int64_t* desc);
+int reduce_plan_one_launch(const int64_t* desc, ReduceMulti* m, int* nblocks);
+}
diff --git a/two-stage-gnn_amd/data_parallel.py b/two-stage-gnn_amd/data_parallel.py
--- a/two-stage-gnn_amd/data_parallel.py
+++ b/two-stage-gnn_amd/data_parallel.py
@@ -28,7 +28,7 @@
         self.numel = off
         self.flat_param = torch.zeros(self.numel, dtype=torch.float32, device=dev)
         self._grad_store = torch.zeros(self.numel + 4, dtype=torch.float32, device=dev)
-        self.flat_grad = self._grad_store[:self.numel]
+        self._flat_grad = self._grad_store[:self.numel]
         self._err_slot = self._grad_store[self.numel:self.numel + 1]
         for p, (o, n) in zip(self.params, self.views):
             self.flat_param[o:o + n].copy_(p.data.reshape(-1))
@@ -51,14 +51,30 @@
         if direct_grads and self.on_gpu:
             self.sink = mp.GradSink()
             for p, (o, n) in zip(self.params, self.views):
-                self.sink.views[p.data_ptr()] = self.flat_grad[o:o + n].view_as(p.data)
+                self.sink.views[p.data_ptr()] = self._flat_grad[o:o + n].view_as(p.data)
             self.sink.norm_parts = torch.zeros(4096, dtype=torch.float32, device=dev)
             self.sink.step_state = self.state
+            self.sink.defer_closing = True
+        self.max_resident = 0
         self.always_reduce = False
         self._early = None
         self._early_issued = False
         self._allow_early = True
         self._side = torch.cuda.Stream() if (self.on_gpu and self.buckets > 1) else None
+
+    def _flush(self):
+        if self.sink is not None:
+            self.sink.flush()
+
+    @property
+    def flat_grad(self):
+        self._flush()
+        return self._flat_grad
+
+    def grad_view(self, param):
+        i = next(k for k, p in enumerate(self.params) if p is param)
+        o, n = self.views[i]
+        return self.flat_grad[o:o + n].view_as(param.data)
 
     def _reducing(self):
         return (self.world > 1 or self.always_reduce) and dist.is_available() and dist.is_initialized()
@@ -85,10 +101,11 @@
             return
         self._side.wait_stream(torch.cuda.current_stream())
         with torch.cuda.stream(self._side):
-            dist.all_reduce(self.flat_grad[rng[0]:rng[1]], op=dist.ReduceOp.SUM, group=self.group)
+            dist.all_reduce(self._flat_grad[rng[0]:rng[1]], op=dist.ReduceOp.SUM, group=self.group)
         self._early_issued = True
 
     def zero_grad(self):
+        self._flush()
         for p in self.params:
             p.grad = None
         self._norm_ready = False
@@ -104,7 +121,11 @@
     def backward(self, loss):
         loss.backward(gradient=mp.unit_seed(loss.device) if loss.is_cuda and loss.dim() == 0 else None)
 
-    def gather_grads(self):
+    def gather_grads(self, flush=True):
+        self._gather_grads()
+        return self.flat_grad if flush else None
+
+    def _gather_grads(self):
         written = ()
         mp.CE_DEFER = False
         if self.sink is not None:
@@ -112,15 +133,17 @@
             written = self.sink.written
             self._norm_ready = (bool(written) and self.sink.stepped and written == self.sink.normed and not self.sink.reused
                                 and all(p.grad is None for p in self.params) and self.world == 1 and not self.always_reduce)
+            if not self._norm_ready:
+                self._flush()
         if not written:
             parts = []
             for p, z, pz in zip(self.params, self._zeros, self._pad_zeros):
                 if pz is not None:
                     parts.append(pz)
                 parts.append(p.grad.reshape(-1) if p.grad is not None else z)
-            torch.cat(parts, out=self.flat_grad)
+            torch.cat(parts, out=self._flat_grad)
             self._dirty = {i for i, p in enumerate(self.params) if p.grad is not None}
-            return self.flat_grad
+            return self._flat_grad
         cp_dst, cp_src, add_dst, add_src, zero_dst = [], [], [], [], []
         for i, (p, (o, n)) in enumerate(zip(self.params, self.views)):
             direct = p.data_ptr() in written
@@ -129,16 +152,16 @@
                     extra = p.grad.reshape(-1).contiguous()
                     dist.all_reduce(extra, op=dist.ReduceOp.SUM, group=self.group)
                     torch.cuda.current_stream().wait_stream(self._side)
-                    self.flat_grad[o:o + n].add_(extra)
+                    self._flat_grad[o:o + n].add_(extra)
                 elif direct:
-                    add_dst.append(self.flat_grad[o:o + n]); add_src.append(p.grad.reshape(-1))
+                    add_dst.append(self._flat_grad[o:o + n]); add_src.append(p.grad.reshape(-1))
                 else:
-                    cp_dst.append(self.flat_grad[o:o + n]); cp_src.append(p.grad.reshape(-1))
+                    cp_dst.append(self._flat_grad[o:o + n]); cp_src.append(p.grad.reshape(-1))
                 self._dirty.add(i)
             elif direct:
                 self._dirty.add(i)
             elif i in self._dirty:
-                zero_dst.append(self.flat_grad[o:o + n])
+                zero_dst.append(self._flat_grad[o:o + n])
                 self._dirty.discard(i)
         if cp_dst:
             torch._foreach_copy_(cp_dst, cp_src)
@@ -146,10 +169,11 @@
             torch._foreach_add_(add_dst, add_src)
         if zero_dst:
             torch._foreach_zero_(zero_dst)
-        return self.flat_grad
+        return self._flat_grad
 
     def all_reduce(self):
         if self.world > 1 or self.always_reduce:
+            self._flush()
             if self.poison is not None:
                 self._err_slot.copy_(self.poison)
             if self._early_issued:
@@ -170,17 +194,31 @@
             raise RuntimeError("FlatTrainer.apply runs the HIP optimiser kernel; parameters must live on the GPU "
                                "(no CPU fallback)")
         if getattr(self, "_norm_ready", False):
-            nat.call("adam_from_partials_f32", self.flat_param, self.flat_grad, self.exp_avg, self.exp_avg_sq, self.numel,
+            pend = self.sink.pending
+            if pend is not None:
+                from .dense_stack import _workspace
+                sets, _, first, step = pend
+                words, err = _workspace(self.flat_param.device)
+                if nat.try_call("wgrad_reduce_adam_f32", *mp._multi_args(sets), self.sink.norm_parts, int(first),
+                                int(self.sink.norm_used), 1 if step is not None else 0, self.flat_param, self._flat_grad, self.exp_avg,
+                                self.exp_avg_sq, self.numel, float(self.lr), float(self.betas[0]), float(self.betas[1]),
+                                float(self.eps), float(self.wd), float(self.clip), self.state, words, err, int(self.max_resident)):
+                    self.sink.pending = None
+                    return
+                self._flush()
+            nat.call("adam_from_partials_f32", self.flat_param, self._flat_grad, self.exp_avg, self.exp_avg_sq, self.numel,
                      float(self.lr), float(self.betas[0]), float(self.betas[1]), float(self.eps), float(self.wd), float(self.clip),
                      self.state, self.sink.norm_parts, int(self.sink.norm_used), self._poison_word())
             return
+        self._flush()
         if self.sink is not None and self.sink.stepped:
             self.state[0] -= 1.0
-        nat.call("clip_adam_step_f32", self.flat_param, self.flat_grad, self.exp_avg, self.exp_avg_sq, self.numel,
+        nat.call("clip_adam_step_f32", self.flat_param, self._flat_grad, self.exp_avg, self.exp_avg_sq, self.numel,
                  float(self.lr), float(self.betas[0]), float(self.betas[1]), float(self.eps), float(self.wd),
                  float(self.clip), float(scale), self.state, self.ws, self._poison_word())
 
     def check(self):
+        self._flush()
         torch.cuda.synchronize()
         skipped = self.on_gpu and float(self.state[3]) != 0.0
         try:
@@ -198,7 +236,7 @@
         self.zero_grad()
         loss = loss_fn()
         self.backward(loss)
-        self.gather_grads()
+        self.gather_grads(flush=False)
         self.all_reduce()
         self.apply()
         return loss
@@ -407,7 +445,7 @@
         tr.zero_grad()
         self.loss = self.loss_fn()
         tr.backward(self.loss)
-        tr.gather_grads()
+        tr.gather_grads(flush=False)
 
     def synchronize(self):
         self.stream.synchronize()
diff --git a/two-stage-gnn_amd/message_passing.py b/two-stage-gnn_amd/message_passing.py
--- a/two-stage-gnn_amd/message_passing.py
+++ b/two-stage-gnn_amd/message_passing.py
@@ -166,6 +166,13 @@
     return normed
 
 
+def _multi_args(chunk):
+    args = []
+    for ws, nslab, K, N, dw, db in list(chunk) + [(None, 0, 0, 0, None, None)] * (4 - len(chunk)):
+        args += [ws, int(nslab), int(K), int(N), dw, db]
+    return args
+
+
 def wgrad_reduce_multi(sets, norm_sink=None):
     normed = norm_sink is not None
     for i in range(0, len(sets), 4):
@@ -173,11 +180,11 @@
         parts, step = (_norm_args(norm_sink, _desc([wgrad_set(*st, kn=1, lddw=st[3]) for st in chunk]))
                        if norm_sink is not None else (None, None))
         normed = normed and parts is not None
-        args = []
-        for ws, nslab, K, N, dw, db in chunk + [(None, 0, 0, 0, None, None)] * (4 - len(chunk)):
-            args += [ws, int(nslab), int(K), int(N), dw, db]
-        nat.call("wgrad_reduce_multi_f32", *args, parts, step)
+        nat.call("wgrad_reduce_multi_f32", *_multi_args(chunk), parts, step)
     return normed
+
+
+CLOSING_LAUNCH = os.environ.get("TSGNN_CLOSING_LAUNCH", "1") != "0"
 
 
 class WgradSets:
@@ -209,6 +216,13 @@
             return
         shares = (self.sink is not None and len(self.params) > 0 and self.all_sunk
                   and (self.max_sets is None or len(self.sets) <= self.max_sets))
+        if (shares and CLOSING_LAUNCH and self.launcher is wgrad_reduce_multi and len(self.sets) <= 4 and nat._defer is None
+                and self.sink.pend(self.sets)):
+            self.sink.normed.update(p.data_ptr() for p in self.params)
+            self.sets = []
+            return
+        if getattr(self.sink, "pending", None) is not None:
+            self.sink.flush()
         if self.launcher(self.sets, norm_sink=self.sink if shares else None):
             self.sink.normed.update(p.data_ptr() for p in self.params)
         self.sets = []
@@ -914,6 +928,8 @@
         self.step_state = None
         self.norm_enabled = False
         self.ready_cb = None
+        self.defer_closing = False
+        self.pending = None
         self.reset_norm()
 
     def ready(self, params):
@@ -925,6 +941,22 @@
         self.normed = set()
         self.stepped = False
         self.reused = False
+
+    def pend(self, sets):
+        if not (self.defer_closing and self.norm_enabled and self.norm_parts is not None) or len(sets) > 4:
+            return False
+        self.flush()
+        first = self.norm_used
+        parts, step = _norm_args(self, _desc([wgrad_set(*st, kn=1, lddw=st[3]) for st in sets]))
+        if parts is None:
+            return False
+        self.pending = (list(sets), parts, first, step)
+        return True
+
+    def flush(self):
+        if self.pending is not None:
+            (sets, parts, _, step), self.pending = self.pending, None
+            nat.call("wgrad_reduce_multi_f32", *_multi_args(sets), parts, step)
 
     def norm_slots(self, n):
         if not self.norm_enabled or self.norm_parts is None or self.norm_used + n > self.norm_parts.numel():
```

Measured after the change: 237,900. 0.921x the previous value.
